# bcaitech1/p4-fr-sorry-math-but-love-you

Hardware: NVIDIA B200
Metric: EfficientSATRN greedy-decode images/sec (higher is better)
Workload: dtype bf16

## Files before the change

### p4-fr-sorry-math-but-love-you_b200/csrc/common.cuh

```cuda
#pragma once
#include <cuda_runtime.h>
#include <cuda_bf16.h>
#include <cuda_fp16.h>
#include <stdint.h>

#if defined(__CUDA_ARCH__) && (__CUDA_ARCH__ < 1000)
#error "frx is written for sm_100a (B200) only"
#endif

namespace frx {

enum Act : int { ACT_NONE = 0, ACT_RELU = 1, ACT_SILU = 2, ACT_SIGMOID = 3, ACT_GELU = 4 };

__device__ __forceinline__ float act_apply(float v, int act) {
  switch (act) {
    case ACT_RELU: return fmaxf(v, 0.f);
    case ACT_SILU: return v / (1.f + expf(-v));
    case ACT_SIGMOID: return 1.f / (1.f + expf(-v));
    case ACT_GELU: return 0.5f * v * (1.f + erff(v * 0.70710678118654752440f));
    default: return v;
  }
}

struct SmemOptIn {
  size_t bytes[64] = {};
  template <class Kernel>
  cudaError_t ensure(Kernel kernel, size_t smem, bool always = false) {
    int dev = 0;
    cudaGetDevice(&dev);
    dev &= 63;
    if ((!always && smem <= 48 * 1024) || (bytes[dev] != 0 && smem <= bytes[dev])) return cudaSuccess;
    cudaError_t e = cudaFuncSetAttribute(kernel, cudaFuncAttributeMaxDynamicSharedMemorySize, (int)smem);
    if (e == cudaSuccess) bytes[dev] = smem;
    return e;
  }
};

#ifndef FRX_ENC_FP16
#define FRX_ENC_FP16 1
#endif
#if FRX_ENC_FP16
typedef __half eh_t;
typedef __half2 eh2_t;
#define FRX_EH_PTX "f16"
__device__ __forceinline__ uint32_t eh2_pack(float lo, float hi) {
  uint32_t r;
  asm("cvt.rn.satfinite.f16x2.f32 %0, %1, %2;\n" : "=r"(r) : "f"(hi), "f"(lo));
  return r;
}
__device__ __forceinline__ eh_t eh_from_float(float f) {
  const uint32_t r = eh2_pack(f, 0.f);
  return __ushort_as_half((unsigned short)(r & 0xffffu));
}
__device__ __forceinline__ float eh_to_float(eh_t v) { return __half2float(v); }
__device__ __forceinline__ float2 eh2_unpack(uint32_t w) { return __half22float2(*reinterpret_cast<const __half2*>(&w)); }
#else
typedef __nv_bfloat16 eh_t;
typedef __nv_bfloat162 eh2_t;
#define FRX_EH_PTX "bf16"
__device__ __forceinline__ uint32_t eh2_pack(float lo, float hi) {
  __nv_bfloat162 t = __floats2bfloat162_rn(lo, hi);
  return *reinterpret_cast<uint32_t*>(&t);
}
__device__ __forceinline__ eh_t eh_from_float(float f) { return __float2bfloat16_rn(f); }
__device__ __forceinline__ float eh_to_float(eh_t v) { return __bfloat162float(v); }
__device__ __forceinline__ float2 eh2_unpack(uint32_t w) { return make_float2(__uint_as_float(w << 16), __uint_as_float(w & 0xffff0000u)); }
#endif

__device__ __forceinline__ float warp_sum(float v) {
#pragma unroll
  for (int o = 16; o > 0; o >>= 1) v += __shfl_xor_sync(0xffffffffu, v, o);
  return v;
}
__device__ __forceinline__ float warp_max(float v) {
#pragma unroll
  for (int o = 16; o > 0; o >>= 1) v = fmaxf(v, __shfl_xor_sync(0xffffffffu, v, o));
  return v;
}

struct GemmP {
  const float* A;
  const float* W;
  float* C;
  int M, N, K;
  int lda, ldc;
  int conv;
  int H, Wd, Cin, OH, OW, KH, KW, stride, pad_t, pad_l;
  const float* gate;
  int rows_per_img;
  const float* scale;
  const float* shift;
  int act;
  const float* res;
  int ldr;
  float* ws;
  long long ws_floats;
  int splitk, k_chunk;
};

struct DwP {
  const float* in;
  const float* w;
  const float* scale;
  const float* shift;
  float* out;
  int B, H, Wd, C, OH, OW, stride, pad_t, pad_l, act;
};

struct Seg {
  int n_begin, n_end;
  float* dst;
  long long row_stride;
  long long slot_stride;
};

struct DecGemmP {
  const float* A;
  const float* Wt;
  const float* bias;
  int M, N, K, lda;
  int act;
  const float* res;
  int ldr;
  const float* ln_g;
  const float* ln_b;
  float* a_norm_out;
  const int* row_slot;
  int nseg;
  Seg seg[4];
};

struct AttnP {
  const float* q;
  int ldq;
  const float* kcache;
  const float* vcache;
  int rows_per_img;
  int D;
  int n_hist;
  const int* hist_len;
  int causal_L;
  const unsigned char* key_mask;
  const int* chain;
  int chain_stride;
  const float* cur_k;
  const float* cur_v;
  int ld_cur;
  int q_per_img;
  float temperature;
  float* out;
  int ldo;
  int M;
  int heads;
};


struct BeamP {
  int B, V, bw, max_seq, T, cap, sos, eos, pad;
  double* hscore; int* hnode; int* hsize;
  int* nprev; int* ntok; int* nlen; double* nlogp; int* nkv; int* ncount;
  int *num_steps, *done, *endnode, *nexp, *cur_node;
  int *cur_tok, *pos, *slot, *active;
  int* chain;
  int* n_active;
  const float* logits;
  long long* out;
};

struct TcGemmP {
  const eh_t* A;
  const eh_t* W;
  void* C;
  int M, N, K, lda, ldw, ldc;
  int BN;
  int stages;
  int conv, H, Wd, Cin, OH, OW, KW, stride, pad_t, pad_l;
  const eh_t* Wpad;
  int im2col;
  const float* scale;
  const float* shift;
  int act;
  const void* res;
  int res_f32, ldr, out_f32;
};

struct SiftIds { int sos, eos, empty, lbrace, rbrace, underbar; };

constexpr int DEC_CLUSTER = 8;
constexpr int DEC_IMG = 8;
constexpr int DEC_FMAX = 1024;
constexpr int DEC_TMAX = 500;
constexpr int DEC_MAX_CLUSTERS = 32;

struct DecClusterLayer {
  const uint4 *w_o, *w_q2, *w_o2, *w_f0, *w_f1, *w_next;
  const float *b_o, *b_q2, *b_o2, *b_f0, *b_f1, *b_next;
  const float *ln1_g, *ln1_b, *ln2_g, *ln2_b, *ln3_g, *ln3_b;
};

struct DecClusterP {
  int B, steps, T, L, V, S, sos;
  int img_base;
  const uint4* w_first;
  const float* b_first;
  DecClusterLayer layer[4];
  const float* emb;
  const float* pe;
  __nv_bfloat16* kself;
  __nv_bfloat16* vself;
  const __nv_bfloat16* kcross;
  const __nv_bfloat16* vcross;
  float* logits;
  long long* tokens;
  const long long* forced;
  const int* hist_len;
  const int* chain;
  const int* slot;
  const int* first_tok32;
  const long long* first_tok64;
  const int* sift_flags;
  const int* sift_limit;
  SiftIds sift_ids;
  long long* prof;
};

}
```

### p4-fr-sorry-math-but-love-you_b200/csrc/kernels.h

```cpp
#pragma once
#include "common.cuh"

namespace frx {

void launch_stem_conv(const float* in, const float* w, const float* scale, const float* shift, float* out,
                      int B, int Cin, int H, int W, int OH, int OW, int Cout, cudaStream_t st);
void launch_direct_conv3x3(const float* in, const float* w, const float* scale, const float* shift, float* out, int B,
                           int Cin, int H, int W, int OH, int OW, int Cout, int stride, int pad, int act,
                           cudaStream_t st);
void launch_igemm_f32(const GemmP& p, cudaStream_t st);
void launch_dwconv_f32(const DwP& p, cudaStream_t st);
void launch_se_gate_f32(const float* x, const float* w1, const float* b1, const float* w2, const float* b2,
                        float* gate, int B, int HW, int C, int R, cudaStream_t st);
void launch_maxpool2_f32(const float* in, float* out, int B, int H, int W, int C, cudaStream_t st);
void launch_pe2d_f32(const float* x, const float* w0, const float* b0, const float* w1, const float* b1,
                     const float* peh, const float* pew, float* out, int B, int h, int w, int C,
                     cudaStream_t st);
void launch_layernorm_f32(const float* x, const float* res, const float* gamma, const float* beta, float* out,
                          int M, int C, int scramble_S, cudaStream_t st);
void launch_enc_attn_f32(const float* qkv, float* out, int B, int S, int D, int heads, cudaStream_t st);
void launch_dec_gemm_f32(const DecGemmP& p, cudaStream_t st);
void launch_dec_attn_f32(const AttnP& p, int head_dim, cudaStream_t st);
void launch_fill_i32(int* p, int v, int n, cudaStream_t st);
void launch_dec_embed_f32(const int* tok, const long long* tok64, int fixed_token, const float* emb,
                          const float* pe, int pos, const int* pos_arr, int pos_mod, float scale, float* x,
                          int M, int D, cudaStream_t st);
void launch_dec_argmax_embed(const float* logits, long long ld_logits, int V, long long* tokens_out,
                             long long ld_tok, const long long* forced, long long ld_forced, int* cur_tok,
                             const float* emb, const float* pe_next, float scale, float* x, int M, int D,
                             cudaStream_t st);


void launch_dec_sift_embed(float* logits, long long ld_logits, int V, long long* tokens_out, long long ld_tok, int4* state,
                           const int* flags, const int* limit, const SiftIds& ids, int* cur_tok, const float* emb,
                           const float* pe_next, float scale, float* x, int M, int D, cudaStream_t st);
void launch_sift_state_init(int4* state, int M, int sos, cudaStream_t st);
void launch_pad_mask(const long long* text, unsigned char* mask, int B, int L, int pad_id, cudaStream_t st);

void launch_swin_patch_embed(const float* img, const float* w, const float* bias, const float* g, const float* b,
                             const float* ape, float* out, int B, int IMGS, int R, int E, cudaStream_t st);
void launch_swin_window_attn(const float* qkv, const float* bias_table, float* out, int B, int R, int C, int heads, int ws,
                             int shift, cudaStream_t st);
bool launch_swin_window_attn_mma(const float* qkv, const float* bias_table, eh_t* out, int B, int R, int C, int heads,
                                 int ws, int shift, cudaStream_t st);
void launch_swin_patch_merge(const float* x, float* out, int B, int R, int C, cudaStream_t st);

void launch_beam_init(const BeamP& p, cudaStream_t st);
void launch_beam_select(const BeamP& p, cudaStream_t st);
void launch_beam_push(const BeamP& p, cudaStream_t st);
void launch_beam_finish(const BeamP& p, cudaStream_t st);

int launch_tc_igemm(TcGemmP p, cudaStream_t st);
int launch_tc_igemm_ws(TcGemmP p, int num_sms, cudaStream_t st);
void launch_pad_conv_weights(const eh_t* in, eh_t* out, long long rows, int Cin, cudaStream_t st);
void launch_h16_to_f32(const eh_t* in, float* out, long long n, cudaStream_t st);
void launch_f32_to_h16(const float* in, eh_t* out, long long n, cudaStream_t st);
void launch_stem_conv_bf16(const float* in, const float* w, const float* scale, const float* shift,
                           eh_t* out, int B, int Cin, int H, int W, int OH, int OW, int Cout, cudaStream_t st);
void launch_dwconv_bf16(const eh_t* in, const float* w, const float* scale, const float* shift,
                        eh_t* out, int B, int H, int W, int C, int OH, int OW, int stride, int pad_t,
                        int pad_l, int act, cudaStream_t st);
void launch_se_scale_bf16(eh_t* x, const float* w1, const float* b1, const float* w2, const float* b2,
                          int B, int HW, int C, int R, cudaStream_t st);
void launch_mbconv_dw_se_bf16(const eh_t* in, const float* w, const float* scale, const float* shift,
                              eh_t* out, float* mean, float* gate, const float* w1, const float* b1,
                              const float* w2, const float* b2, int B, int H, int W, int C, int OH, int OW, int stride,
                              int pad_t, int pad_l, int R, cudaStream_t st);
void launch_layernorm_bf16out(const float* x, const float* res, const float* gamma, const float* beta,
                              eh_t* out, int M, int C, int scramble_S, cudaStream_t st);
void launch_enc_attn_bf16out(const float* qkv, eh_t* out, int B, int S, int D, int heads, cudaStream_t st);
void launch_conv3x3_c24_bf16(const eh_t* in, const void* wfrag, const float* scale, const float* shift,
                             eh_t* out, int B, int H, int W, int add_res, cudaStream_t st);
void launch_lite_conv0_pool_bf16(const float* in, const float* w, const float* scale, const float* shift, eh_t* out,
                                 int B, int Cin, int H, int W, int Cout, cudaStream_t st);
void launch_maxpool2_bf16(const eh_t* in, eh_t* out, float* out_f32, int B, int H, int W, int C, cudaStream_t st);
bool launch_enc_attn_mma_bf16(const float* qkv, eh_t* out, int B, int S, int D, int heads, cudaStream_t st);

size_t dec_cluster_smem_bytes();
int launch_dec_cluster_bf16(const DecClusterP& p, cudaStream_t st);
int launch_dec_cluster_bf16_d128(const DecClusterP& p, cudaStream_t st);
int launch_dec_cluster_bf16_p2(const DecClusterP& p, cudaStream_t st);
int launch_dec_cluster_bf16_d512(const DecClusterP& p, cudaStream_t st);
void launch_cross_to_bf16(const float* src, __nv_bfloat16* kc, __nv_bfloat16* vc, int B, int S, int L, int Dm, int head_dim,
                          cudaStream_t st);

}
```

### p4-fr-sorry-math-but-love-you_b200/csrc/kernels_bf16.cu

```cuda
#include <cuda_fp16.h>

#include "common.cuh"
#include "kernels.h"

#ifndef FRX_DW_ACC32
#define FRX_DW_ACC32 2
#endif

namespace frx {

namespace {
__device__ __forceinline__ void unpack8(const uint4& u, float (&f)[8]) {
  const uint32_t w[4] = {u.x, u.y, u.z, u.w};
#pragma unroll
  for (int i = 0; i < 4; ++i) {
    const float2 t = eh2_unpack(w[i]);
    f[2 * i] = t.x;
    f[2 * i + 1] = t.y;
  }
}
__device__ __forceinline__ uint4 pack8(const float (&f)[8]) {
  uint32_t w[4];
#pragma unroll
  for (int i = 0; i < 4; ++i) w[i] = eh2_pack(f[2 * i], f[2 * i + 1]);
  return make_uint4(w[0], w[1], w[2], w[3]);
}
}

__global__ void __launch_bounds__(256) stem_conv_bf16_kernel(const float* __restrict__ in, const float* __restrict__ w,
                                                             const float* __restrict__ scale, const float* __restrict__ shift,
                                                             eh_t* __restrict__ out, int B, int Cin, int H, int W,
                                                             int OH, int OW, int Cout) {
  extern __shared__ float ws[];
  for (int i = threadIdx.x; i < Cout * Cin * 9; i += blockDim.x) ws[i] = w[i];
  float* ssc = ws + Cout * Cin * 9;
  float* ssh = ssc + Cout;
  for (int i = threadIdx.x; i < Cout; i += blockDim.x) { ssc[i] = scale[i]; ssh[i] = shift[i]; }
  __syncthreads();
  const int C8 = Cout / 8;
  long long total = (long long)B * OH * OW * C8;
  long long idx = (long long)blockIdx.x * blockDim.x + threadIdx.x;
  if (idx >= total) return;
  const int co0 = (int)(idx % C8) * 8;
  long long pix = idx / C8;
  const int ow = (int)(pix % OW), oh = (int)((pix / OW) % OH), n = (int)(pix / ((long long)OW * OH));
  float acc[8];
#pragma unroll
  for (int j = 0; j < 8; ++j) acc[j] = 0.f;
  for (int ci = 0; ci < Cin; ++ci) {
    const float* ip = in + (((long long)n * Cin + ci) * H + oh * 2) * W + ow * 2;
    float x[9];
#pragma unroll
    for (int kh = 0; kh < 3; ++kh)
#pragma unroll
      for (int kw = 0; kw < 3; ++kw) x[kh * 3 + kw] = __ldg(ip + kh * W + kw);
#pragma unroll
    for (int j = 0; j < 8; ++j) {
      const float* wp = ws + ((co0 + j) * Cin + ci) * 9;
#pragma unroll
      for (int t = 0; t < 9; ++t) acc[j] = fmaf(x[t], wp[t], acc[j]);
    }
  }
  float o[8];
#pragma unroll
  for (int j = 0; j < 8; ++j) o[j] = act_apply(acc[j] * ssc[co0 + j] + ssh[co0 + j], ACT_SILU);
  *reinterpret_cast<uint4*>(out + pix * Cout + co0) = pack8(o);
}

template <int COUT>
__global__ void __launch_bounds__(128) stem_conv_px_bf16_kernel(const float* __restrict__ in, const float* __restrict__ w,
                                                                const float* __restrict__ scale, const float* __restrict__ shift,
                                                                eh_t* __restrict__ out, int B, int Cin, int H, int W,
                                                                int OH, int OW) {
  extern __shared__ __align__(16) float ws[];
  const int taps = Cin * 9;
  for (int i = threadIdx.x; i < COUT * taps; i += blockDim.x) {
    const int co = i / taps, r = i - co * taps;
    ws[r * COUT + co] = w[i];
  }
  float* ssc = ws + COUT * taps;
  float* ssh = ssc + COUT;
  uint4* stage = reinterpret_cast<uint4*>(ws + ((COUT * taps + 2 * COUT + 3) & ~3));
  for (int i = threadIdx.x; i < COUT; i += blockDim.x) { ssc[i] = scale[i]; ssh[i] = shift[i]; }
  __syncthreads();
  const long long npix = (long long)B * OH * OW, pix0 = (long long)blockIdx.x * blockDim.x;
  const long long pix = min(pix0 + threadIdx.x, npix - 1);
  const int ow = (int)(pix % OW), oh = (int)((pix / OW) % OH), n = (int)(pix / ((long long)OW * OH));
  float acc[COUT];
#pragma unroll
  for (int j = 0; j < COUT; ++j) acc[j] = 0.f;
  for (int ci = 0; ci < Cin; ++ci) {
    const float* ip = in + (((long long)n * Cin + ci) * H + oh * 2) * W + ow * 2;
    float x[9];
#pragma unroll
    for (int kh = 0; kh < 3; ++kh)
#pragma unroll
      for (int kw = 0; kw < 3; ++kw) x[kh * 3 + kw] = __ldg(ip + kh * W + kw);
#pragma unroll
    for (int t = 0; t < 9; ++t) {
      const float4* wp = reinterpret_cast<const float4*>(ws + (ci * 9 + t) * COUT);
#pragma unroll
      for (int j = 0; j < COUT / 4; ++j) {
        const float4 wv = wp[j];
        acc[4 * j] = fmaf(x[t], wv.x, acc[4 * j]);
        acc[4 * j + 1] = fmaf(x[t], wv.y, acc[4 * j + 1]);
        acc[4 * j + 2] = fmaf(x[t], wv.z, acc[4 * j + 2]);
        acc[4 * j + 3] = fmaf(x[t], wv.w, acc[4 * j + 3]);
      }
    }
  }
#pragma unroll
  for (int g = 0; g < COUT / 8; ++g) {
    float o[8];
#pragma unroll
    for (int j = 0; j < 8; ++j) o[j] = act_apply(acc[g * 8 + j] * ssc[g * 8 + j] + ssh[g * 8 + j], ACT_SILU);
    stage[threadIdx.x * (COUT / 8) + g] = pack8(o);
  }
  __syncthreads();
  const long long cta_vecs = min((long long)blockDim.x, npix - pix0) * (COUT / 8);
  uint4* op = reinterpret_cast<uint4*>(out + pix0 * COUT);
  for (int i = threadIdx.x; i < cta_vecs; i += blockDim.x) op[i] = stage[i];
}

void launch_stem_conv_bf16(const float* in, const float* w, const float* scale, const float* shift,
                           eh_t* out, int B, int Cin, int H, int W, int OH, int OW, int Cout, cudaStream_t st) {
  if (Cout == 24) {
    const long long pixels = (long long)B * OH * OW;
    const int smem24 = ((24 * Cin * 9 + 2 * 24 + 3) & ~3) * sizeof(float) + 128 * 3 * 16;
    stem_conv_px_bf16_kernel<24><<<(unsigned)((pixels + 127) / 128), 128, smem24, st>>>(in, w, scale, shift, out, B, Cin, H, W, OH, OW);
    return;
  }
  long long total = (long long)B * OH * OW * (Cout / 8);
  int smem = (Cout * Cin * 9 + 2 * Cout) * sizeof(float);
  stem_conv_bf16_kernel<<<(unsigned)((total + 255) / 256), 256, smem, st>>>(in, w, scale, shift, out, B, Cin, H, W, OH, OW, Cout);
}

__global__ void __launch_bounds__(256) dwconv3x3_bf16_kernel(const eh_t* __restrict__ in, const float* __restrict__ w,
                                                             const float* __restrict__ scale, const float* __restrict__ shift,
                                                             eh_t* __restrict__ out, int B, int H, int W, int C, int OH,
                                                             int OW, int stride, int pad_t, int pad_l, int act) {
  const int C8 = C >> 3;
  long long total = (long long)B * OH * OW * C8;
  long long idx = (long long)blockIdx.x * blockDim.x + threadIdx.x;
  if (idx >= total) return;
  const int c = (int)(idx % C8) * 8;
  long long pix = idx / C8;
  const int ow = (int)(pix % OW), oh = (int)((pix / OW) % OH), n = (int)(pix / ((long long)OW * OH));
  float acc[8];
#pragma unroll
  for (int j = 0; j < 8; ++j) acc[j] = 0.f;
#pragma unroll
  for (int kh = 0; kh < 3; ++kh) {
    const int ih = oh * stride - pad_t + kh;
    if (ih < 0 || ih >= H) continue;
#pragma unroll
    for (int kw = 0; kw < 3; ++kw) {
      const int iw = ow * stride - pad_l + kw;
      if (iw < 0 || iw >= W) continue;
      float x[8];
      unpack8(__ldg(reinterpret_cast<const uint4*>(in + (((long long)n * H + ih) * W + iw) * C + c)), x);
      const float4 w0 = __ldg(reinterpret_cast<const float4*>(w + (kh * 3 + kw) * C + c));
      const float4 w1 = __ldg(reinterpret_cast<const float4*>(w + (kh * 3 + kw) * C + c + 4));
      acc[0] = fmaf(x[0], w0.x, acc[0]); acc[1] = fmaf(x[1], w0.y, acc[1]);
      acc[2] = fmaf(x[2], w0.z, acc[2]); acc[3] = fmaf(x[3], w0.w, acc[3]);
      acc[4] = fmaf(x[4], w1.x, acc[4]); acc[5] = fmaf(x[5], w1.y, acc[5]);
      acc[6] = fmaf(x[6], w1.z, acc[6]); acc[7] = fmaf(x[7], w1.w, acc[7]);
    }
  }
  float o[8];
#pragma unroll
  for (int j = 0; j < 8; ++j) o[j] = act_apply(acc[j] * __ldg(scale + c + j) + __ldg(shift + c + j), act);
  *reinterpret_cast<uint4*>(out + pix * C + c) = pack8(o);
}

void launch_dwconv_bf16(const eh_t* in, const float* w, const float* scale, const float* shift,
                        eh_t* out, int B, int H, int W, int C, int OH, int OW, int stride, int pad_t,
                        int pad_l, int act, cudaStream_t st) {
  long long total = (long long)B * OH * OW * (C / 8);
  dwconv3x3_bf16_kernel<<<(unsigned)((total + 255) / 256), 256, 0, st>>>(in, w, scale, shift, out, B, H, W, C, OH, OW,
                                                                        stride, pad_t, pad_l, act);
}

__global__ void __launch_bounds__(256) se_scale_bf16_kernel(eh_t* __restrict__ x, const float* __restrict__ w1,
                                                            const float* __restrict__ b1, const float* __restrict__ w2,
                                                            const float* __restrict__ b2, int HW, int C, int R) {
  extern __shared__ float sm[];
  float* mean = sm;
  float* red = sm + C;
  float* gate = red + R;
  const int n = blockIdx.x;
  eh_t* xp = x + (long long)n * HW * C;
  const float inv = 1.f / (float)HW;
  for (int c8 = threadIdx.x; c8 < C / 8; c8 += blockDim.x) {
    float s[8];
#pragma unroll
    for (int j = 0; j < 8; ++j) s[j] = 0.f;
    for (int q = 0; q < HW; ++q) {
      float v[8];
      unpack8(*reinterpret_cast<const uint4*>(xp + (long long)q * C + c8 * 8), v);
#pragma unroll
      for (int j = 0; j < 8; ++j) s[j] += v[j];
    }
#pragma unroll
    for (int j = 0; j < 8; ++j) mean[c8 * 8 + j] = s[j] * inv;
  }
  __syncthreads();
  const int warp = threadIdx.x >> 5, lane = threadIdx.x & 31;
  for (int r = warp; r < R; r += 8) {
    float s = 0.f;
    for (int c = lane; c < C; c += 32) s = fmaf(__ldg(w1 + (long long)r * C + c), mean[c], s);
    s = warp_sum(s);
    if (lane == 0) red[r] = act_apply(s + __ldg(b1 + r), ACT_SILU);
  }
  __syncthreads();
  for (int c = threadIdx.x; c < C; c += blockDim.x) {
    float s = __ldg(b2 + c);
    const float* wr = w2 + (long long)c * R;
    for (int r = 0; r < R; ++r) s = fmaf(__ldg(wr + r), red[r], s);
    gate[c] = 1.f / (1.f + expf(-s));
  }
  __syncthreads();
  for (int i = threadIdx.x; i < HW * (C / 8); i += blockDim.x) {
    const int c8 = i % (C / 8);
    uint4* ptr = reinterpret_cast<uint4*>(xp + (long long)(i / (C / 8)) * C + c8 * 8);
    float v[8];
    unpack8(*ptr, v);
#pragma unroll
    for (int j = 0; j < 8; ++j) v[j] *= gate[c8 * 8 + j];
    *ptr = pack8(v);
  }
}

void launch_se_scale_bf16(eh_t* x, const float* w1, const float* b1, const float* w2, const float* b2,
                          int B, int HW, int C, int R, cudaStream_t st) {
  se_scale_bf16_kernel<<<B, 256, (2 * C + R) * sizeof(float), st>>>(x, w1, b1, w2, b2, HW, C, R);
}


__global__ void __launch_bounds__(256) dwconv_se_mean_kernel(const eh_t* __restrict__ in, const float* __restrict__ w,
                                                             const float* __restrict__ scale, const float* __restrict__ shift,
                                                             eh_t* __restrict__ out, float* __restrict__ mean,
                                                             int H, int W, int C, int OH, int OW, int stride, int pad_t,
                                                             int pad_l, const float* __restrict__ se_w1,
                                                             const float* __restrict__ se_w2, int se_floats) {
  extern __shared__ __align__(16) unsigned char dw_smem[];
  {
    const long long line = ((long long)(blockIdx.y * gridDim.x + blockIdx.x) * blockDim.x + threadIdx.x) * 32;
    if (line < se_floats) {
      asm volatile("prefetch.global.L2 [%0];\n" ::"l"(se_w1 + line));
      asm volatile("prefetch.global.L2 [%0];\n" ::"l"(se_w2 + line));
    }
  }
  uint4* tile = reinterpret_cast<uint4*>(dw_smem);
  float (*red)[64 + 1] = reinterpret_cast<float (*)[64 + 1]>(dw_smem + (size_t)H * W * 8 * 16);
  float* wsm = reinterpret_cast<float*>(dw_smem + (size_t)H * W * 8 * 16 + 32 * 65 * sizeof(float));
  const int n = blockIdx.x, c0 = blockIdx.y * 64;
  const int cg = threadIdx.x & 7, pl = threadIdx.x >> 3;
  const int c = c0 + cg * 8;
  const bool c_ok = c < C;
  const eh_t* ip = in + (long long)n * H * W * C;
  for (int i = threadIdx.x; i < H * W * 8; i += 256) {
    const int px = i >> 3, g = i & 7;
    tile[i] = (c0 + g * 8 < C) ? __ldg(reinterpret_cast<const uint4*>(ip + (long long)px * C + c0 + g * 8)) : make_uint4(0u, 0u, 0u, 0u);
  }
  float sum[8];
#pragma unroll
  for (int j = 0; j < 8; ++j) sum[j] = 0.f;
  for (int i = threadIdx.x; i < 11 * 64; i += 256) {
    const int t = i >> 6, cc = c0 + (i & 63);
    const float* src = t < 9 ? w + t * C : (t == 9 ? scale : shift);
    wsm[i] = cc < C ? __ldg(src + cc) : 0.f;
  }
  __syncthreads();
  auto ld8s = [&](int t, float (&dst)[8]) {
    const float4 a = *reinterpret_cast<const float4*>(wsm + t * 64 + cg * 8);
    const float4 b4 = *reinterpret_cast<const float4*>(wsm + t * 64 + cg * 8 + 4);
    dst[0] = a.x; dst[1] = a.y; dst[2] = a.z; dst[3] = a.w; dst[4] = b4.x; dst[5] = b4.y; dst[6] = b4.z; dst[7] = b4.w;
  };
  float sc[8], sh[8];
  ld8s(9, sc);
  ld8s(10, sh);
  eh_t* op = out + (long long)n * OH * OW * C;
  if (c_ok) {
    for (int px = pl; px < OH * OW; px += 32) {
      const int oh = px / OW, ow = px - oh * OW;
      float acc[8];
#pragma unroll
      for (int j = 0; j < 8; ++j) acc[j] = 0.f;
#pragma unroll
      for (int kh = 0; kh < 3; ++kh) {
        const int ih = oh * stride - pad_t + kh;
#pragma unroll
        for (int kw = 0; kw < 3; ++kw) {
          const int iw = ow * stride - pad_l + kw;
          if (ih >= 0 && ih < H && iw >= 0 && iw < W) {
            float x[8], wv[8];
            unpack8(tile[(ih * W + iw) * 8 + cg], x);
            ld8s(kh * 3 + kw, wv);
#pragma unroll
            for (int j = 0; j < 8; ++j) acc[j] = fmaf(x[j], wv[j], acc[j]);
          }
        }
      }
      float o[8];
#pragma unroll
      for (int j = 0; j < 8; ++j) {
        const float v = fmaf(acc[j], sc[j], sh[j]);
        o[j] = __fdividef(v, 1.f + __expf(-v));
      }
      const uint4 packed = pack8(o);
      *reinterpret_cast<uint4*>(op + (long long)px * C + c) = packed;
      float back[8];
      unpack8(packed, back);
#pragma unroll
      for (int j = 0; j < 8; ++j) sum[j] += back[j];
    }
  }
#pragma unroll
  for (int j = 0; j < 8; ++j) red[pl][cg * 8 + j] = sum[j];
  __syncthreads();
  if (threadIdx.x < 64 && c0 + threadIdx.x < C) {
    float s = 0.f;
#pragma unroll
    for (int i = 0; i < 32; ++i) s += red[i][threadIdx.x];
    mean[(long long)n * C + c0 + threadIdx.x] = s / (float)(OH * OW);
  }
}

template <int CH>
__global__ void __launch_bounds__(CH * 4) dwconv4_se_mean_kernel(const eh_t* __restrict__ in, const float* __restrict__ w,
                                                                 const float* __restrict__ scale, const float* __restrict__ shift,
                                                                 eh_t* __restrict__ out, float* __restrict__ mean,
                                                                 int H, int W, int C, int OH, int OW, int stride, int pad_t,
                                                                 int pad_l, const float* __restrict__ se_w1,
                                                                 const float* __restrict__ se_w2, int se_floats) {
  constexpr int NT = CH * 4, G8 = CH / 8, G4 = CH / 4;
  extern __shared__ __align__(16) unsigned char dw_smem[];
  {
    const long long line = ((long long)(blockIdx.y * gridDim.x + blockIdx.x) * NT + threadIdx.x) * 32;
    if (line < se_floats) {
      asm volatile("prefetch.global.L2 [%0];\n" ::"l"(se_w1 + line));
      asm volatile("prefetch.global.L2 [%0];\n" ::"l"(se_w2 + line));
    }
  }
  uint4* tile = reinterpret_cast<uint4*>(dw_smem);
  float (*red)[CH + 1] = reinterpret_cast<float (*)[CH + 1]>(dw_smem + (size_t)H * W * G8 * 16);
  const int n = blockIdx.x, c0 = blockIdx.y * CH;
  const eh_t* ip = in + (long long)n * H * W * C;
  for (int i = threadIdx.x; i < H * W * G8; i += NT) {
    const int px = i / G8, g = i - px * G8;
    uint4 v = make_uint4(0u, 0u, 0u, 0u);
    if (c0 + g * 8 < C) {
#if FRX_ENC_FP16
      v = __ldg(reinterpret_cast<const uint4*>(ip + (long long)px * C + c0 + g * 8));
#else
      float x[8];
      unpack8(__ldg(reinterpret_cast<const uint4*>(ip + (long long)px * C + c0 + g * 8)), x);
      const __half2 h0 = __floats2half2_rn(x[0], x[1]), h1 = __floats2half2_rn(x[2], x[3]);
      const __half2 h2 = __floats2half2_rn(x[4], x[5]), h3 = __floats2half2_rn(x[6], x[7]);
      v = make_uint4(*reinterpret_cast<const uint32_t*>(&h0), *reinterpret_cast<const uint32_t*>(&h1),
                     *reinterpret_cast<const uint32_t*>(&h2), *reinterpret_cast<const uint32_t*>(&h3));
#endif
    }
    tile[i] = v;
  }
  const int cg = threadIdx.x % G4, pl = threadIdx.x / G4;
  const int c = c0 + cg * 4;
  const bool c_ok = c < C;
#if FRX_DW_ACC32
  float4 wt[9], sc, sh;
#if FRX_DW_ACC32 == 2
  __half2 wh[9][2];
#endif
  {
    const float4 z = make_float4(0.f, 0.f, 0.f, 0.f);
#pragma unroll
    for (int t = 0; t < 9; ++t) wt[t] = c_ok ? __ldg(reinterpret_cast<const float4*>(w + t * C + c)) : z;
#if FRX_DW_ACC32 == 2
#pragma unroll
    for (int t = 0; t < 9; ++t) { wh[t][0] = __floats2half2_rn(wt[t].x, wt[t].y); wh[t][1] = __floats2half2_rn(wt[t].z, wt[t].w); }
#endif
    sc = c_ok ? __ldg(reinterpret_cast<const float4*>(scale + c)) : z;
    sh = c_ok ? __ldg(reinterpret_cast<const float4*>(shift + c)) : z;
  }
  __syncthreads();
  const uint2* tile2 = reinterpret_cast<const uint2*>(tile);
  float sum[4] = {0.f, 0.f, 0.f, 0.f};
  eh_t* op = out + (long long)n * OH * OW * C;
  if (c_ok) {
    for (int px = pl; px < OH * OW; px += 16) {
      const int oh = px / OW, ow = px - oh * OW;
      float4 acc = make_float4(0.f, 0.f, 0.f, 0.f);
#pragma unroll
      for (int kh = 0; kh < 3; ++kh) {
        const int ih = oh * stride - pad_t + kh;
#if FRX_DW_ACC32 == 2
        __half2 r0 = __floats2half2_rn(0.f, 0.f), r1 = r0;
#pragma unroll
        for (int kw = 0; kw < 3; ++kw) {
          const int iw = ow * stride - pad_l + kw;
          if (ih >= 0 && ih < H && iw >= 0 && iw < W) {
            const uint2 u = tile2[(ih * W + iw) * G4 + cg];
            r0 = __hfma2(*reinterpret_cast<const __half2*>(&u.x), wh[kh * 3 + kw][0], r0);
            r1 = __hfma2(*reinterpret_cast<const __half2*>(&u.y), wh[kh * 3 + kw][1], r1);
          }
        }
        const float2 a = __half22float2(r0), b = __half22float2(r1);
        acc.x += a.x; acc.y += a.y; acc.z += b.x; acc.w += b.y;
#else
#pragma unroll
        for (int kw = 0; kw < 3; ++kw) {
          const int iw = ow * stride - pad_l + kw;
          if (ih >= 0 && ih < H && iw >= 0 && iw < W) {
            const uint2 u = tile2[(ih * W + iw) * G4 + cg];
            const float2 a = __half22float2(*reinterpret_cast<const __half2*>(&u.x)), b = __half22float2(*reinterpret_cast<const __half2*>(&u.y));
            const float4 ww = wt[kh * 3 + kw];
            acc.x = fmaf(a.x, ww.x, acc.x); acc.y = fmaf(a.y, ww.y, acc.y); acc.z = fmaf(b.x, ww.z, acc.z); acc.w = fmaf(b.y, ww.w, acc.w);
          }
        }
#endif
      }
      float2 f0 = make_float2(fmaf(acc.x, sc.x, sh.x), fmaf(acc.y, sc.y, sh.y)), f1 = make_float2(fmaf(acc.z, sc.z, sh.z), fmaf(acc.w, sc.w, sh.w));
      f0.x = __fdividef(f0.x, 1.f + __expf(-f0.x)); f0.y = __fdividef(f0.y, 1.f + __expf(-f0.y));
      f1.x = __fdividef(f1.x, 1.f + __expf(-f1.x)); f1.y = __fdividef(f1.y, 1.f + __expf(-f1.y));
#else
  __half2 wt[9][2], sc[2], sh[2];
  {
    const float4 z = make_float4(0.f, 0.f, 0.f, 0.f);
#pragma unroll
    for (int t = 0; t < 9; ++t) {
      const float4 f = c_ok ? __ldg(reinterpret_cast<const float4*>(w + t * C + c)) : z;
      wt[t][0] = __floats2half2_rn(f.x, f.y); wt[t][1] = __floats2half2_rn(f.z, f.w);
    }
    const float4 a = c_ok ? __ldg(reinterpret_cast<const float4*>(scale + c)) : z;
    const float4 d = c_ok ? __ldg(reinterpret_cast<const float4*>(shift + c)) : z;
    sc[0] = __floats2half2_rn(a.x, a.y); sc[1] = __floats2half2_rn(a.z, a.w);
    sh[0] = __floats2half2_rn(d.x, d.y); sh[1] = __floats2half2_rn(d.z, d.w);
  }
  const __half2 half_ = __floats2half2_rn(0.5f, 0.5f);
  __syncthreads();
  const uint2* tile2 = reinterpret_cast<const uint2*>(tile);
  float sum[4] = {0.f, 0.f, 0.f, 0.f};
  eh_t* op = out + (long long)n * OH * OW * C;
  if (c_ok) {
    for (int px = pl; px < OH * OW; px += 16) {
      const int oh = px / OW, ow = px - oh * OW;
      __half2 acc0 = __floats2half2_rn(0.f, 0.f), acc1 = acc0;
#pragma unroll
      for (int kh = 0; kh < 3; ++kh) {
        const int ih = oh * stride - pad_t + kh;
#pragma unroll
        for (int kw = 0; kw < 3; ++kw) {
          const int iw = ow * stride - pad_l + kw;
          if (ih >= 0 && ih < H && iw >= 0 && iw < W) {
            const uint2 u = tile2[(ih * W + iw) * G4 + cg];
            acc0 = __hfma2(*reinterpret_cast<const __half2*>(&u.x), wt[kh * 3 + kw][0], acc0);
            acc1 = __hfma2(*reinterpret_cast<const __half2*>(&u.y), wt[kh * 3 + kw][1], acc1);
          }
        }
      }
      const __half2 v0 = __hfma2(acc0, sc[0], sh[0]), v1 = __hfma2(acc1, sc[1], sh[1]);
      const __half2 o0 = __hmul2(v0, __hfma2(h2tanh_approx(__hmul2(v0, half_)), half_, half_));
      const __half2 o1 = __hmul2(v1, __hfma2(h2tanh_approx(__hmul2(v1, half_)), half_, half_));
      const float2 f0 = __half22float2(o0), f1 = __half22float2(o1);
#endif
      uint2 packed;
      packed.x = eh2_pack(f0.x, f0.y);
      packed.y = eh2_pack(f1.x, f1.y);
      *reinterpret_cast<uint2*>(op + (long long)px * C + c) = packed;
      const float2 b0 = eh2_unpack(packed.x), b1 = eh2_unpack(packed.y);
      sum[0] += b0.x; sum[1] += b0.y; sum[2] += b1.x; sum[3] += b1.y;
    }
  }
#pragma unroll
  for (int j = 0; j < 4; ++j) red[pl][cg * 4 + j] = sum[j];
  __syncthreads();
  if (threadIdx.x < CH && c0 + threadIdx.x < C) {
    float s2 = 0.f;
#pragma unroll
    for (int i = 0; i < 16; ++i) s2 += red[i][threadIdx.x];
    mean[(long long)n * C + c0 + threadIdx.x] = s2 / (float)(OH * OW);
  }
}

constexpr int SE_IMGS = 4;
constexpr int SE_ROWS = 4;
__global__ void __launch_bounds__(512, 1) se_fc_kernel(const float* __restrict__ mean, const float* __restrict__ w1,
                                                       const float* __restrict__ b1, const float* __restrict__ w2,
                                                       const float* __restrict__ b2, float* __restrict__ gate, int B, int C,
                                                       int R) {
  extern __shared__ float sm[];
  float* mv = sm;
  float* red = sm + SE_IMGS * C;
  const int n0 = blockIdx.x * SE_IMGS;
  for (int i = threadIdx.x; i < SE_IMGS * C; i += blockDim.x) {
    const int im = i / C;
    mv[i] = n0 + im < B ? mean[(long long)n0 * C + i] : 0.f;
  }
  __syncthreads();
  const int warp = threadIdx.x >> 5, lane = threadIdx.x & 31;
  const int nwarps = blockDim.x >> 5;
  for (int r0 = warp * SE_ROWS; r0 < R; r0 += nwarps * SE_ROWS) {
    float s[SE_ROWS][SE_IMGS];
#pragma unroll
    for (int j = 0; j < SE_ROWS; ++j)
#pragma unroll
      for (int im = 0; im < SE_IMGS; ++im) s[j][im] = 0.f;
#pragma unroll 3
    for (int c4 = lane; c4 < C / 4; c4 += 32) {
      float4 wv[SE_ROWS], m4[SE_IMGS];
#pragma unroll
      for (int j = 0; j < SE_ROWS; ++j)
        wv[j] = r0 + j < R ? __ldg(reinterpret_cast<const float4*>(w1 + (long long)(r0 + j) * C) + c4) : make_float4(0.f, 0.f, 0.f, 0.f);
#pragma unroll
      for (int im = 0; im < SE_IMGS; ++im) m4[im] = *reinterpret_cast<const float4*>(mv + im * C + c4 * 4);
#pragma unroll
      for (int j = 0; j < SE_ROWS; ++j)
#pragma unroll
        for (int im = 0; im < SE_IMGS; ++im)
          s[j][im] = fmaf(wv[j].x, m4[im].x, fmaf(wv[j].y, m4[im].y, fmaf(wv[j].z, m4[im].z, fmaf(wv[j].w, m4[im].w, s[j][im]))));
    }
#pragma unroll
    for (int j = 0; j < SE_ROWS; ++j)
#pragma unroll
      for (int im = 0; im < SE_IMGS; ++im) {
        const float t = warp_sum(s[j][im]);
        if (lane == 0 && r0 + j < R) red[im * R + r0 + j] = act_apply(t + __ldg(b1 + r0 + j), ACT_SILU);
      }
  }
  __syncthreads();
  for (int c = blockIdx.y * blockDim.x + threadIdx.x; c < C; c += gridDim.y * blockDim.x) {
    float s[SE_IMGS];
    const float bb = __ldg(b2 + c);
#pragma unroll
    for (int im = 0; im < SE_IMGS; ++im) s[im] = bb;
#pragma unroll 32
    for (int r = 0; r < R; ++r) {
      const float wv = __ldg(w2 + (long long)r * C + c);
#pragma unroll
      for (int im = 0; im < SE_IMGS; ++im) s[im] = fmaf(wv, red[im * R + r], s[im]);
    }
#pragma unroll
    for (int im = 0; im < SE_IMGS; ++im)
      if (n0 + im < B) gate[(long long)(n0 + im) * C + c] = 1.f / (1.f + expf(-s[im]));
  }
}

__global__ void __launch_bounds__(256) se_apply_kernel(eh_t* __restrict__ x, const float* __restrict__ gate,
                                                       long long total8, int HW, int C) {
  long long i = (long long)blockIdx.x * blockDim.x + threadIdx.x;
  if (i >= total8) return;
  const int C8 = C >> 3;
  const int c = (int)(i % C8) * 8;
  const long long n = i / ((long long)C8 * HW);
  uint4* ptr = reinterpret_cast<uint4*>(x) + i;
  float v[8];
  unpack8(*ptr, v);
  const float4 g0 = __ldg(reinterpret_cast<const float4*>(gate + n * C + c));
  const float4 g1 = __ldg(reinterpret_cast<const float4*>(gate + n * C + c + 4));
  v[0] *= g0.x; v[1] *= g0.y; v[2] *= g0.z; v[3] *= g0.w;
  v[4] *= g1.x; v[5] *= g1.y; v[6] *= g1.z; v[7] *= g1.w;
  *ptr = pack8(v);
}

void launch_mbconv_dw_se_bf16(const eh_t* in, const float* w, const float* scale, const float* shift,
                              eh_t* out, float* mean, float* gate, const float* w1, const float* b1,
                              const float* w2, const float* b2, int B, int H, int W, int C, int OH, int OW, int stride,
                              int pad_t, int pad_l, int R, cudaStream_t st) {
  dim3 g(B, (C + 63) / 64);
  const size_t smem = (size_t)H * W * 8 * 16 + 32 * 65 * sizeof(float) + 11 * 64 * sizeof(float);
  static SmemOptIn opt;
  opt.ensure(dwconv_se_mean_kernel, smem);
  if (C % 8 == 0) {
    constexpr int CH = 32;
    const size_t sm4 = (size_t)H * W * (CH / 8) * 16 + 16 * (CH + 1) * sizeof(float);
    static SmemOptIn opt4;
    opt4.ensure(dwconv4_se_mean_kernel<CH>, sm4);
    dwconv4_se_mean_kernel<CH><<<dim3(B, (C + CH - 1) / CH), CH * 4, sm4, st>>>(in, w, scale, shift, out, mean, H, W, C, OH, OW,
                                                                             stride, pad_t, pad_l, w1, w2, R * C);
  } else {
    dwconv_se_mean_kernel<<<g, 256, smem, st>>>(in, w, scale, shift, out, mean, H, W, C, OH, OW, stride, pad_t, pad_l, w1, w2, R * C);
  }
  se_fc_kernel<<<dim3((B + SE_IMGS - 1) / SE_IMGS, 2), 512, SE_IMGS * (C + R) * sizeof(float), st>>>(mean, w1, b1, w2, b2, gate, B, C, R);
  long long total8 = (long long)B * OH * OW * (C / 8);
  se_apply_kernel<<<(unsigned)((total8 + 255) / 256), 256, 0, st>>>(out, gate, total8, OH * OW, C);
}

__device__ __forceinline__ uint32_t pack2(float lo, float hi) {
  return eh2_pack(lo, hi);
}
__device__ __forceinline__ void mma16816(float (&c)[4], const uint32_t (&a)[4], uint32_t b0, uint32_t b1) {
  asm("mma.sync.aligned.m16n8k16.row.col.f32." FRX_EH_PTX "." FRX_EH_PTX ".f32 {%0,%1,%2,%3}, {%4,%5,%6,%7}, {%8,%9}, {%0,%1,%2,%3};\n"
      : "+f"(c[0]), "+f"(c[1]), "+f"(c[2]), "+f"(c[3])
      : "r"(a[0]), "r"(a[1]), "r"(a[2]), "r"(a[3]), "r"(b0), "r"(b1));
}

template <int S>
__global__ void __launch_bounds__(S * 2) enc_attn_mma_kernel(const float* __restrict__ qkv,
                                                             eh_t* __restrict__ out,
                                                             int D, int heads, float inv_temp) {
  constexpr int HD = 64, NT = S / 8;
  const int b = blockIdx.x / heads, hh = blockIdx.x % heads;
  const int warp = threadIdx.x >> 5, lane = threadIdx.x & 31, gid = lane >> 2, tig = lane & 3;
  const int ld = 3 * D;
  const float* qb = qkv + (long long)b * S * ld + hh * HD;
  const int i0 = warp * 16;
  float sacc[NT][4];
#pragma unroll
  for (int nt = 0; nt < NT; ++nt)
#pragma unroll
    for (int e = 0; e < 4; ++e) sacc[nt][e] = 0.f;
#pragma unroll
  for (int ks = 0; ks < 4; ++ks) {
    const float* q0 = qb + (long long)(i0 + gid) * ld + 16 * ks + 2 * tig;
    const float* q1 = q0 + 8 * ld;
    const float2 a00 = __ldg(reinterpret_cast<const float2*>(q0)), a10 = __ldg(reinterpret_cast<const float2*>(q1));
    const float2 a01 = __ldg(reinterpret_cast<const float2*>(q0 + 8)), a11 = __ldg(reinterpret_cast<const float2*>(q1 + 8));
    const uint32_t a[4] = {pack2(a00.x, a00.y), pack2(a10.x, a10.y), pack2(a01.x, a01.y), pack2(a11.x, a11.y)};
#pragma unroll
    for (int nt = 0; nt < NT; ++nt) {
      const float* kp = qb + D + (long long)(8 * nt + gid) * ld + 16 * ks + 2 * tig;
      const float2 k0 = __ldg(reinterpret_cast<const float2*>(kp)), k1 = __ldg(reinterpret_cast<const float2*>(kp + 8));
      mma16816(sacc[nt], a, pack2(k0.x, k0.y), pack2(k1.x, k1.y));
    }
  }
  float mx0 = -INFINITY, mx1 = -INFINITY;
#pragma unroll
  for (int nt = 0; nt < NT; ++nt) {
#pragma unroll
    for (int e = 0; e < 4; ++e) sacc[nt][e] *= inv_temp;
    mx0 = fmaxf(mx0, fmaxf(sacc[nt][0], sacc[nt][1]));
    mx1 = fmaxf(mx1, fmaxf(sacc[nt][2], sacc[nt][3]));
  }
  mx0 = fmaxf(mx0, __shfl_xor_sync(0xffffffffu, mx0, 1)); mx0 = fmaxf(mx0, __shfl_xor_sync(0xffffffffu, mx0, 2));
  mx1 = fmaxf(mx1, __shfl_xor_sync(0xffffffffu, mx1, 1)); mx1 = fmaxf(mx1, __shfl_xor_sync(0xffffffffu, mx1, 2));
  float sum0 = 0.f, sum1 = 0.f;
#pragma unroll
  for (int nt = 0; nt < NT; ++nt) {
    sacc[nt][0] = __expf(sacc[nt][0] - mx0); sacc[nt][1] = __expf(sacc[nt][1] - mx0);
    sacc[nt][2] = __expf(sacc[nt][2] - mx1); sacc[nt][3] = __expf(sacc[nt][3] - mx1);
    sum0 += sacc[nt][0] + sacc[nt][1];
    sum1 += sacc[nt][2] + sacc[nt][3];
  }
  sum0 += __shfl_xor_sync(0xffffffffu, sum0, 1); sum0 += __shfl_xor_sync(0xffffffffu, sum0, 2);
  sum1 += __shfl_xor_sync(0xffffffffu, sum1, 1); sum1 += __shfl_xor_sync(0xffffffffu, sum1, 2);
  float oacc[8][4];
#pragma unroll
  for (int n = 0; n < 8; ++n)
#pragma unroll
    for (int e = 0; e < 4; ++e) oacc[n][e] = 0.f;
#pragma unroll
  for (int kk = 0; kk < S / 16; ++kk) {
    const uint32_t a[4] = {pack2(sacc[2 * kk][0], sacc[2 * kk][1]), pack2(sacc[2 * kk][2], sacc[2 * kk][3]),
                           pack2(sacc[2 * kk + 1][0], sacc[2 * kk + 1][1]), pack2(sacc[2 * kk + 1][2], sacc[2 * kk + 1][3])};
    const float* vp = qb + 2 * D + (long long)(16 * kk + 2 * tig) * ld + gid;
#pragma unroll
    for (int n = 0; n < 8; ++n) {
      const float v00 = __ldg(vp + 8 * n), v01 = __ldg(vp + ld + 8 * n);
      const float v10 = __ldg(vp + 8 * ld + 8 * n), v11 = __ldg(vp + 9 * ld + 8 * n);
      mma16816(oacc[n], a, pack2(v00, v01), pack2(v10, v11));
    }
  }
  const float r0 = __fdividef(1.f, sum0), r1 = __fdividef(1.f, sum1);
  eh_t* o0 = out + ((long long)b * S + i0 + gid) * D + hh * HD + 2 * tig;
  eh_t* o1 = o0 + (long long)8 * D;
#pragma unroll
  for (int n = 0; n < 8; ++n) {
    *reinterpret_cast<uint32_t*>(o0 + 8 * n) = pack2(oacc[n][0] * r0, oacc[n][1] * r0);
    *reinterpret_cast<uint32_t*>(o1 + 8 * n) = pack2(oacc[n][2] * r1, oacc[n][3] * r1);
  }
}

bool launch_enc_attn_mma_bf16(const float* qkv, eh_t* out, int B, int S, int D, int heads, cudaStream_t st) {
  if (D / heads != 64 || D % heads != 0) return false;
  const float inv_temp = 1.f / sqrtf((float)D);
  if (S == 32) enc_attn_mma_kernel<32><<<B * heads, 64, 0, st>>>(qkv, out, D, heads, inv_temp);
  else if (S == 128) enc_attn_mma_kernel<128><<<B * heads, 256, 0, st>>>(qkv, out, D, heads, inv_temp);
  else return false;
  return true;
}

constexpr int C24 = 24, C24_TH = 8, C24_TW = 32, C24_KS = 14;

__global__ void __launch_bounds__(256) conv3x3_c24_mma_kernel(const eh_t* __restrict__ in, const uint2* __restrict__ wfrag,
                                                              const float* __restrict__ scale, const float* __restrict__ shift,
                                                              eh_t* __restrict__ out, int H, int W, int add_res) {
  constexpr int PW = C24_TW + 2, PH = C24_TH + 2;
  __shared__ __align__(16) eh_t halo[PH * PW * C24];
  __shared__ uint2 wsm[C24_KS * 3 * 32];
  const int tiles_x = (W + C24_TW - 1) / C24_TW, tiles_y = (H + C24_TH - 1) / C24_TH;
  const int n = blockIdx.x / (tiles_x * tiles_y), t = blockIdx.x % (tiles_x * tiles_y);
  const int y0 = (t / tiles_x) * C24_TH, x0 = (t % tiles_x) * C24_TW;
  const eh_t* ip = in + (long long)n * H * W * C24;
  for (int i = threadIdx.x; i < PH * PW * 3; i += 256) {
    const int pix = i / 3, ch = i - pix * 3;
    const int py = pix / PW, px = pix - py * PW;
    const int y = y0 + py - 1, x = x0 + px - 1;
    uint4 v = make_uint4(0u, 0u, 0u, 0u);
    if (y >= 0 && y < H && x >= 0 && x < W) v = __ldg(reinterpret_cast<const uint4*>(ip + ((long long)y * W + x) * C24) + ch);
    reinterpret_cast<uint4*>(halo)[i] = v;
  }
  for (int i = threadIdx.x; i < C24_KS * 3 * 32; i += 256) wsm[i] = __ldg(wfrag + i);
  __syncthreads();
  const int warp = threadIdx.x >> 5, lane = threadIdx.x & 31, gid = lane >> 2, tig = lane & 3;
  float acc[2][3][4];
#pragma unroll
  for (int mt = 0; mt < 2; ++mt)
#pragma unroll
    for (int nt = 0; nt < 3; ++nt)
#pragma unroll
      for (int e = 0; e < 4; ++e) acc[mt][nt][e] = 0.f;
  const uint32_t* hw = reinterpret_cast<const uint32_t*>(halo);
#pragma unroll
  for (int s = 0; s < C24_KS; ++s) {
    const int klo = 16 * s, khi = 16 * s + 8;
    const int tap_lo = klo / C24, ch_lo = klo % C24, tap_hi = khi / C24, ch_hi = khi % C24;
    uint32_t a[2][4];
#pragma unroll
    for (int mt = 0; mt < 2; ++mt) {
      const int px = mt * 16 + gid;
      const int p_lo = ((warp + tap_lo / 3) * PW + px + tap_lo % 3) * 12 + (ch_lo >> 1) + tig;
      a[mt][0] = hw[p_lo];
      a[mt][1] = hw[p_lo + 8 * 12];
      if (tap_hi < 9) {
        const int p_hi = ((warp + tap_hi / 3) * PW + px + tap_hi % 3) * 12 + (ch_hi >> 1) + tig;
        a[mt][2] = hw[p_hi];
        a[mt][3] = hw[p_hi + 8 * 12];
      } else {
        a[mt][2] = 0u; a[mt][3] = 0u;
      }
    }
#pragma unroll
    for (int nt = 0; nt < 3; ++nt) {
      const uint2 b = wsm[(s * 3 + nt) * 32 + lane];
      mma16816(acc[0][nt], a[0], b.x, b.y);
      mma16816(acc[1][nt], a[1], b.x, b.y);
    }
  }
  const int y = y0 + warp;
  if (y >= H) return;
  eh_t* op = out + ((long long)n * H + y) * W * C24;
#pragma unroll
  for (int nt = 0; nt < 3; ++nt) {
    const int ch = nt * 8 + 2 * tig;
    const float s0 = __ldg(scale + ch), s1 = __ldg(scale + ch + 1), h0 = __ldg(shift + ch), h1 = __ldg(shift + ch + 1);
#pragma unroll
    for (int mt = 0; mt < 2; ++mt)
#pragma unroll
      for (int hr = 0; hr < 2; ++hr) {
        const int px = mt * 16 + gid + hr * 8, x = x0 + px;
        if (x >= W) continue;
        float v0 = fmaf(acc[mt][nt][2 * hr], s0, h0), v1 = fmaf(acc[mt][nt][2 * hr + 1], s1, h1);
        v0 = __fdividef(v0, 1.f + __expf(-v0));
        v1 = __fdividef(v1, 1.f + __expf(-v1));
        if (add_res) {
          const uint32_t r = hw[((warp + 1) * PW + px + 1) * 12 + (ch >> 1)];
          const float2 rf = eh2_unpack(r);
          v0 += rf.x;
          v1 += rf.y;
        }
        *reinterpret_cast<uint32_t*>(op + (long long)x * C24 + ch) = pack2(v0, v1);
      }
  }
}

void launch_conv3x3_c24_bf16(const eh_t* in, const void* wfrag, const float* scale, const float* shift,
                             eh_t* out, int B, int H, int W, int add_res, cudaStream_t st) {
  const int tiles = ((W + C24_TW - 1) / C24_TW) * ((H + C24_TH - 1) / C24_TH);
  conv3x3_c24_mma_kernel<<<B * tiles, 256, 0, st>>>(in, reinterpret_cast<const uint2*>(wfrag), scale, shift, out, H, W, add_res);
}

__global__ void __launch_bounds__(256) lite_conv0_pool_bf16_kernel(const float* __restrict__ in, const float* __restrict__ w,
                                                                   const float* __restrict__ scale, const float* __restrict__ shift,
                                                                   eh_t* __restrict__ out, int B, int Cin, int H, int W, int Cout) {
  extern __shared__ float ws0[];
  for (int i = threadIdx.x; i < Cout * Cin * 9; i += blockDim.x) ws0[i] = w[i];
  float* ssc = ws0 + Cout * Cin * 9;
  float* ssh = ssc + Cout;
  for (int i = threadIdx.x; i < Cout; i += blockDim.x) { ssc[i] = scale[i]; ssh[i] = shift[i]; }
  __syncthreads();
  const int OH = H / 2, OW = W / 2, C8 = Cout / 8;
  const long long total = (long long)B * OH * OW * C8;
  const long long idx = (long long)blockIdx.x * blockDim.x + threadIdx.x;
  if (idx >= total) return;
  const int co0 = (int)(idx % C8) * 8;
  const long long pix = idx / C8;
  const int ow = (int)(pix % OW), oh = (int)((pix / OW) % OH), n = (int)(pix / ((long long)OW * OH));
  float acc[4][8];
#pragma unroll
  for (int q = 0; q < 4; ++q)
#pragma unroll
    for (int j = 0; j < 8; ++j) acc[q][j] = 0.f;
  for (int ci = 0; ci < Cin; ++ci) {
    float x[4][4];
#pragma unroll
    for (int a = 0; a < 4; ++a)
#pragma unroll
      for (int b = 0; b < 4; ++b) {
        const int ih = 2 * oh - 1 + a, iw = 2 * ow - 1 + b;
        x[a][b] = (ih >= 0 && ih < H && iw >= 0 && iw < W) ? __ldg(in + (((long long)n * Cin + ci) * H + ih) * W + iw) : 0.f;
      }
#pragma unroll
    for (int j = 0; j < 8; ++j) {
      const float* wp = ws0 + ((co0 + j) * Cin + ci) * 9;
#pragma unroll
      for (int kh = 0; kh < 3; ++kh)
#pragma unroll
        for (int kw = 0; kw < 3; ++kw) {
          const float wv = wp[kh * 3 + kw];
          acc[0][j] = fmaf(x[kh][kw], wv, acc[0][j]);
          acc[1][j] = fmaf(x[kh][kw + 1], wv, acc[1][j]);
          acc[2][j] = fmaf(x[kh + 1][kw], wv, acc[2][j]);
          acc[3][j] = fmaf(x[kh + 1][kw + 1], wv, acc[3][j]);
        }
    }
  }
  float o[8];
#pragma unroll
  for (int j = 0; j < 8; ++j) {
    const float s = ssc[co0 + j], t = ssh[co0 + j];
    const float m = fmaxf(fmaxf(fmaf(acc[0][j], s, t), fmaf(acc[1][j], s, t)), fmaxf(fmaf(acc[2][j], s, t), fmaf(acc[3][j], s, t)));
    o[j] = fmaxf(m, 0.f);
  }
  *reinterpret_cast<uint4*>(out + pix * Cout + co0) = pack8(o);
}

template <int KS, int Cout>
__global__ void __launch_bounds__(256) lite_conv0_pool_mma_kernel(const float* __restrict__ in, const float* __restrict__ w,
                                                                  const float* __restrict__ scale, const float* __restrict__ shift,
                                                                  eh_t* __restrict__ out, int B, int Cin, int H, int W) {
  constexpr int NT = Cout / 8;
  const int lane = threadIdx.x & 31, gid = lane >> 2, tig = lane & 3;
  const int OH = H / 2, OW = W / 2, K = 9 * Cin;
  const long long tiles = (long long)B * OH * (OW / 4);
  const long long tile = (long long)blockIdx.x * 8 + (threadIdx.x >> 5);
  if (tile >= tiles) return;
  uint32_t bf[KS][NT][2];
#pragma unroll
  for (int ks = 0; ks < KS; ++ks)
#pragma unroll
    for (int nt = 0; nt < NT; ++nt)
#pragma unroll
      for (int h2 = 0; h2 < 2; ++h2) {
        const int k = 16 * ks + 8 * h2 + 2 * tig, n = 8 * nt + gid;
        const float lo = k < K ? __ldg(w + (long long)n * K + k) : 0.f, hi = k + 1 < K ? __ldg(w + (long long)n * K + k + 1) : 0.f;
        bf[ks][nt][h2] = pack2(lo, hi);
      }
  const int owq = (int)(tile % (OW / 4));
  const long long t2 = tile / (OW / 4);
  const int oh = (int)(t2 % OH), n = (int)(t2 / OH);
  const int pp = gid & 3, pos0 = gid >> 2;
  const int ow = owq * 4 + pp;
  const float* img = in + (long long)n * Cin * H * W;
  auto patch = [&](int pos, int k) -> float {
    if (k >= K) return 0.f;
    const int ci = k / 9, tap = k - ci * 9, kh = tap / 3, kw = tap - kh * 3;
    const int ih = 2 * oh + (pos >> 1) + kh - 1, iw = 2 * ow + (pos & 1) + kw - 1;
    return (ih >= 0 && ih < H && iw >= 0 && iw < W) ? __ldg(img + ((long long)ci * H + ih) * W + iw) : 0.f;
  };
  float acc[NT][4];
#pragma unroll
  for (int nt = 0; nt < NT; ++nt)
#pragma unroll
    for (int e = 0; e < 4; ++e) acc[nt][e] = 0.f;
#pragma unroll
  for (int ks = 0; ks < KS; ++ks) {
    const int k0 = 16 * ks + 2 * tig;
    const uint32_t a[4] = {pack2(patch(pos0, k0), patch(pos0, k0 + 1)), pack2(patch(pos0 + 2, k0), patch(pos0 + 2, k0 + 1)),
                           pack2(patch(pos0, k0 + 8), patch(pos0, k0 + 9)), pack2(patch(pos0 + 2, k0 + 8), patch(pos0 + 2, k0 + 9))};
#pragma unroll
    for (int nt = 0; nt < NT; ++nt) mma16816(acc[nt], a, bf[ks][nt][0], bf[ks][nt][1]);
  }
  eh_t* op = out + (((long long)n * OH + oh) * OW + ow) * Cout;
#pragma unroll
  for (int nt = 0; nt < NT; ++nt) {
    const int ch = 8 * nt + 2 * tig;
    const float s0 = __ldg(scale + ch), s1 = __ldg(scale + ch + 1), t0 = __ldg(shift + ch), t1 = __ldg(shift + ch + 1);
    float m0 = fmaxf(fmaf(acc[nt][0], s0, t0), fmaf(acc[nt][2], s0, t0));
    float m1 = fmaxf(fmaf(acc[nt][1], s1, t1), fmaf(acc[nt][3], s1, t1));
    m0 = fmaxf(m0, __shfl_xor_sync(0xffffffffu, m0, 16));
    m1 = fmaxf(m1, __shfl_xor_sync(0xffffffffu, m1, 16));
    if (gid < 4) *reinterpret_cast<uint32_t*>(op + ch) = pack2(fmaxf(m0, 0.f), fmaxf(m1, 0.f));
  }
}

void launch_lite_conv0_pool_bf16(const float* in, const float* w, const float* scale, const float* shift, eh_t* out,
                                 int B, int Cin, int H, int W, int Cout, cudaStream_t st) {
  if ((Cout == 64 || Cout == 128) && Cin <= 3 && (W / 2) % 4 == 0 && H % 2 == 0) {
    const long long tiles = (long long)B * (H / 2) * (W / 2 / 4);
    const unsigned grid = (unsigned)((tiles + 7) / 8);
    if (Cout == 64) {
      if (Cin == 1) lite_conv0_pool_mma_kernel<1, 64><<<grid, 256, 0, st>>>(in, w, scale, shift, out, B, Cin, H, W);
      else lite_conv0_pool_mma_kernel<2, 64><<<grid, 256, 0, st>>>(in, w, scale, shift, out, B, Cin, H, W);
    } else {
      if (Cin == 1) lite_conv0_pool_mma_kernel<1, 128><<<grid, 256, 0, st>>>(in, w, scale, shift, out, B, Cin, H, W);
      else lite_conv0_pool_mma_kernel<2, 128><<<grid, 256, 0, st>>>(in, w, scale, shift, out, B, Cin, H, W);
    }
    return;
  }
  const long long total = (long long)B * (H / 2) * (W / 2) * (Cout / 8);
  const int smem = (Cout * Cin * 9 + 2 * Cout) * sizeof(float);
  lite_conv0_pool_bf16_kernel<<<(unsigned)((total + 255) / 256), 256, smem, st>>>(in, w, scale, shift, out, B, Cin, H, W, Cout);
}

__global__ void __launch_bounds__(256) maxpool2_bf16_kernel(const eh_t* __restrict__ in, eh_t* __restrict__ out,
                                                            float* __restrict__ out_f32, int B, int H, int W, int C) {
  const int OH = H / 2, OW = W / 2, C8 = C / 8;
  const long long total = (long long)B * OH * OW * C8;
  const long long idx = (long long)blockIdx.x * blockDim.x + threadIdx.x;
  if (idx >= total) return;
  const int c = (int)(idx % C8) * 8;
  const long long pix = idx / C8;
  const int ow = (int)(pix % OW), oh = (int)((pix / OW) % OH), n = (int)(pix / ((long long)OW * OH));
  const eh_t* base = in + (((long long)n * H + oh * 2) * W + ow * 2) * C + c;
  float a[8], b[8], d[8], e[8], o[8];
  unpack8(__ldg(reinterpret_cast<const uint4*>(base)), a);
  unpack8(__ldg(reinterpret_cast<const uint4*>(base + C)), b);
  unpack8(__ldg(reinterpret_cast<const uint4*>(base + (long long)W * C)), d);
  unpack8(__ldg(reinterpret_cast<const uint4*>(base + (long long)W * C + C)), e);
#pragma unroll
  for (int j = 0; j < 8; ++j) o[j] = fmaxf(fmaxf(a[j], b[j]), fmaxf(d[j], e[j]));
  if (out_f32) {
    float4* op = reinterpret_cast<float4*>(out_f32 + pix * C + c);
    op[0] = make_float4(o[0], o[1], o[2], o[3]);
    op[1] = make_float4(o[4], o[5], o[6], o[7]);
  } else {
    *reinterpret_cast<uint4*>(out + pix * C + c) = pack8(o);
  }
}

void launch_maxpool2_bf16(const eh_t* in, eh_t* out, float* out_f32, int B, int H, int W, int C, cudaStream_t st) {
  const long long total = (long long)B * (H / 2) * (W / 2) * (C / 8);
  maxpool2_bf16_kernel<<<(unsigned)((total + 255) / 256), 256, 0, st>>>(in, out, out_f32, B, H, W, C);
}

}
```

### p4-fr-sorry-math-but-love-you_b200/csrc/kernels_tc.cu

```cuda
#include <cuda.h>
#include <cuda_fp16.h>
#include <cudaTypedefs.h>

#include <cstdio>
#include <cstdlib>

#include "common.cuh"
#include "kernels.h"

namespace frx {

namespace {

constexpr int TC_BM = 128;
constexpr int TC_BK = 64;
constexpr int TC_STAGES = 3;
constexpr int TC_A_BYTES = TC_BM * TC_BK * 2;

__device__ __forceinline__ uint32_t smem_u32(const void* p) { return (uint32_t)__cvta_generic_to_shared(p); }

__device__ __forceinline__ void cp_async16(uint32_t dst, const void* src, uint32_t src_bytes) {
  asm volatile("cp.async.cg.shared.global [%0], [%1], 16, %2;\n" ::"r"(dst), "l"(src), "r"(src_bytes) : "memory");
}
__device__ __forceinline__ void cp_async_commit() { asm volatile("cp.async.commit_group;\n" ::: "memory"); }
// ... 233 lines not shown
  __shared__ uint32_t tmem_base_s;

  const int tid = threadIdx.x, warp = tid >> 5, lane = tid & 31;
  const int BN = p.BN;
  const uint32_t b_bytes = (uint32_t)BN * (TC_BK * 2);
  const uint32_t stage_bytes = TC_A_BYTES + b_bytes;
  const int NS = p.stages;
  const uint32_t smem0 = (smem_u32(dyn_smem) + 1023u) & ~1023u;
  const int m0 = blockIdx.x * TC_BM, n0 = blockIdx.y * BN;
  const int KB = (p.K + TC_BK - 1) / TC_BK;

  if (warp == 0) {
    asm volatile("tcgen05.alloc.cta_group::1.sync.aligned.shared::cta.b32 [%0], %1;\n" ::"r"(smem_u32(&tmem_base_s)), "n"(NCOLS) : "memory");
    asm volatile("tcgen05.relinquish_alloc_permit.cta_group::1.sync.aligned;\n" ::: "memory");
  }
  if (tid == 32) {
#pragma unroll
    for (int s = 0; s < TC_STAGES; ++s) mbar_init(&mma_done[s], 1);
    mbar_init(&acc_done, 1);
    asm volatile("fence.mbarrier_init.release.cluster;\n" ::: "memory");
  }
  tc_fence_before();
  __syncthreads();
  tc_fence_after();
  const uint32_t tmem = tmem_base_s;

  const int c = tid & 7, rbase = tid >> 3;
  const eh_t* a_ptr[4];
  int a_ih0[4], a_iw0[4];
  bool a_ok[4];
#pragma unroll
  for (int i = 0; i < 4; ++i) {
    const int m = m0 + rbase + 32 * i;
    a_ok[i] = m < p.M;
    a_ih0[i] = a_iw0[i] = 0;
    a_ptr[i] = p.A;
    if (a_ok[i]) {
      if (p.conv) {
        const int ow = m % p.OW;
        const int t = m / p.OW;
        const int oh = t % p.OH;
        const int n = t / p.OH;
        a_ptr[i] = p.A + (size_t)n * p.H * p.Wd * p.Cin;
        a_ih0[i] = oh * p.stride - p.pad_t;
        a_iw0[i] = ow * p.stride - p.pad_l;
      } else {
        a_ptr[i] = p.A + (size_t)m * p.lda;
      }
    }
  }
  const int nb_rows = (BN + 31) / 32;

  auto load_stage = [&](int kb, int stage) {
    const uint32_t sa = smem0 + (uint32_t)stage * stage_bytes;
    const uint32_t sb = sa + TC_A_BYTES;
    const int k = kb * TC_BK + c * 8;
    int tap = 0, ci = k, kh = 0, kw = 0;
    if (p.conv) {
      tap = k / p.Cin;
      ci = k - tap * p.Cin;
      kh = tap / p.KW;
      kw = tap - kh * p.KW;
    }
#pragma unroll
    for (int i = 0; i < 4; ++i) {
      const int row = rbase + 32 * i;
      const uint32_t dst = sa + (uint32_t)(row >> 3) * 1024u + (uint32_t)(row & 7) * 128u + (uint32_t)((c ^ (row & 7)) << 4);
      const eh_t* src = p.A;
      uint32_t bytes = 0;
      if (a_ok[i] && k < p.K) {
        if (p.conv) {
          const int ih = a_ih0[i] + kh, iw = a_iw0[i] + kw;
          if (ih >= 0 && ih < p.H && iw >= 0 && iw < p.Wd) {
            src = a_ptr[i] + ((size_t)ih * p.Wd + iw) * p.Cin + ci;
            bytes = 16;
          }
        } else {
          src = a_ptr[i] + k;
          bytes = 16;
        }
      }
      cp_async16(dst, src, bytes);
    }
    for (int j = 0; j < nb_rows; ++j) {
      const int row = rbase + 32 * j;
      if (row < BN) {
        const uint32_t dst = sb + (uint32_t)(row >> 3) * 1024u + (uint32_t)(row & 7) * 128u + (uint32_t)((c ^ (row & 7)) << 4);
        const int n = n0 + row;
        const bool ok = n < p.N && k < p.K;
        cp_async16(dst, ok ? p.W + (size_t)n * p.ldw + k : p.W, ok ? 16u : 0u);
      }
    }
  };

  for (int s = 0; s < NS - 1; ++s) {
    if (s < KB) load_stage(s, s);
    cp_async_commit();
  }
  const uint32_t idesc = make_idesc(BN);
  for (int kb = 0; kb < KB; ++kb) {
    if (NS == 3) cp_async_wait<1>(); else cp_async_wait<0>();
    asm volatile("fence.proxy.async.shared::cta;\n" ::: "memory");
    __syncthreads();
    const int stage = kb % NS;
    if (tid == 0) {
      tc_fence_after();
      const uint32_t sa = smem0 + (uint32_t)stage * stage_bytes;
      const uint64_t adesc = make_smem_desc(sa), bdesc = make_smem_desc(sa + TC_A_BYTES);
#pragma unroll
      for (int j = 0; j < TC_BK / 16; ++j)
        umma_f16(tmem, adesc + (uint64_t)(2 * j), bdesc + (uint64_t)(2 * j), idesc, (kb | j) ? 1u : 0u);
      umma_commit(&mma_done[stage]);
      if (kb == KB - 1) umma_commit(&acc_done);
    }
    const int nk = kb + NS - 1;
    if (nk < KB) {
      if (kb >= 1) mbar_wait(&mma_done[(kb - 1) % NS], (uint32_t)(((kb - 1) / NS) & 1));
      load_stage(nk, nk % NS);
    }
    cp_async_commit();
  }
  cp_async_wait<0>();
  mbar_wait(&acc_done, 0);
  tc_fence_after();

  {
    const int q = warp & 3;
    const int m = m0 + q * 32 + lane;
    const bool m_ok = m < p.M;
    for (int cc = (warp >> 2); cc * 16 < BN; cc += 2) {
      uint32_t r[16];
      tmem_ld16(tmem + ((uint32_t)(q * 32) << 16) + (uint32_t)(cc * 16), r);
      const int nb = n0 + cc * 16;
      if (m_ok && nb < p.N) epilogue_store16<false>(p, r, m, nb);
    }
  }
  tc_fence_before();
  __syncthreads();
  if (warp == 0) {
    asm volatile("tcgen05.dealloc.cta_group::1.sync.aligned.b32 %0, %1;\n" ::"r"(tmem), "n"(NCOLS) : "memory");
  }
}


constexpr int WS_STAGES = 4;
constexpr int WS_LAG = 2;
constexpr int WS_PROD_WARPS = 8;
constexpr int WS_EPI_WARPS = 8;
constexpr int WS_MMA_WARP = WS_PROD_WARPS + WS_EPI_WARPS;
constexpr int WS_TMA_WARP = WS_MMA_WARP + 1;
constexpr int WS_THREADS = (WS_TMA_WARP + 1) * 32;
constexpr int WS_PROD_THREADS = WS_PROD_WARPS * 32;
constexpr int WS_ROWS_PER_PASS = WS_PROD_THREADS / 8;
constexpr int WS_A_PASSES = TC_BM / WS_ROWS_PER_PASS;

template <int NCOLS, bool GELU>
__global__ void __launch_bounds__(WS_THREADS, NCOLS >= 256 ? 1 : 2) tc_igemm_ws_kernel(const TcGemmP p, const __grid_constant__ CUtensorMap tmA,
                                                                  const __grid_constant__ CUtensorMap tmW) {
  extern __shared__ unsigned char dyn_smem[];
  __shared__ __align__(8) uint64_t full_bar[WS_STAGES], empty_bar[WS_STAGES], acc_full[2], acc_empty[2];
  __shared__ uint32_t tmem_base_s;

  const int tid = threadIdx.x, warp = tid >> 5, lane = tid & 31;
  const int BN = p.BN;
  const uint32_t stage_bytes = TC_A_BYTES + (uint32_t)BN * (TC_BK * 2);
  const uint32_t smem0 = (smem_u32(dyn_smem) + 1023u) & ~1023u;
  const int KB = p.im2col ? p.KW * p.KW : (p.K + TC_BK - 1) / TC_BK;
  const int tiles_n = (p.N + BN - 1) / BN;
  const int tiles_m = (p.M + TC_BM - 1) / TC_BM;
  const int num_tiles = tiles_m * tiles_n;
  const bool gather = p.conv && !p.im2col;

  if (warp == WS_MMA_WARP) {
    asm volatile("tcgen05.alloc.cta_group::1.sync.aligned.shared::cta.b32 [%0], %1;\n" ::"r"(smem_u32(&tmem_base_s)), "n"(NCOLS) : "memory");
    asm volatile("tcgen05.relinquish_alloc_permit.cta_group::1.sync.aligned;\n" ::: "memory");
  }
  if (tid == 0) {
#pragma unroll
    for (int s = 0; s < WS_STAGES; ++s) { mbar_init(&full_bar[s], (gather ? WS_PROD_THREADS : 0) + 1); mbar_init(&empty_bar[s], 1); }
    mbar_init(&acc_full[0], 1); mbar_init(&acc_full[1], 1);
    const int epi_threads = (WS_EPI_WARPS + (gather ? 0 : WS_PROD_WARPS)) * 32;
    mbar_init(&acc_empty[0], epi_threads); mbar_init(&acc_empty[1], epi_threads);
    asm volatile("fence.mbarrier_init.release.cluster;\n" ::: "memory");
  }
  tc_fence_before();
  __syncthreads();
  tc_fence_after();
  const uint32_t tmem = tmem_base_s;

  if (gather ? warp < WS_PROD_WARPS : warp == WS_TMA_WARP) {
    const bool tma_thread = gather ? tid == 0 : lane == 0;
    const uint32_t tma_bytes = (uint32_t)BN * (TC_BK * 2) + (gather ? 0u : (uint32_t)TC_A_BYTES);
    if (!gather && !tma_thread) {
    } else {
    const int c = tid & 7, rbase = tid >> 3;
    int it = 0;
    for (int tile = blockIdx.x; tile < num_tiles; tile += gridDim.x) {
      const int m0 = (tile / tiles_n) * TC_BM, n0 = (tile % tiles_n) * BN;
      const eh_t* a_ptr[WS_A_PASSES];
      int a_ih0[WS_A_PASSES], a_iw0[WS_A_PASSES];
      bool a_ok[WS_A_PASSES];
      int bw = 0, bh = 0, bn = 0;
      if (p.im2col) {
        const int ow = m0 % p.OW, tq = m0 / p.OW;
        bw = ow * p.stride - p.pad_l;
        bh = (tq % p.OH) * p.stride - p.pad_t;
        bn = tq / p.OH;
      }
      if (gather) {
#pragma unroll
        for (int i = 0; i < WS_A_PASSES; ++i) {
          const int m = m0 + rbase + WS_ROWS_PER_PASS * i;
          a_ok[i] = m < p.M;
          a_ih0[i] = a_iw0[i] = 0;
          a_ptr[i] = p.A;
          if (a_ok[i]) {
            const int ow = m % p.OW;
            const int tq = m / p.OW;
            const int oh = tq % p.OH;
            const int n = tq / p.OH;
            a_ptr[i] = p.A + (size_t)n * p.H * p.Wd * p.Cin;
            a_ih0[i] = oh * p.stride - p.pad_t;
            a_iw0[i] = ow * p.stride - p.pad_l;
          }
        }
      }
      for (int kb = 0; kb < KB; ++kb, ++it) {
        const int stage = it % WS_STAGES;
        mbar_wait(&empty_bar[stage], (uint32_t)(((it / WS_STAGES) & 1) ^ 1));
        const uint32_t sa = smem0 + (uint32_t)stage * stage_bytes, sb = sa + TC_A_BYTES;
        if (tma_thread) {
          mbar_arrive_expect_tx(&full_bar[stage], tma_bytes);
          tma_load_2d(sb, &tmW, kb * TC_BK, n0, &full_bar[stage]);
          if (p.im2col) tma_load_im2col(sa, &tmA, 0, bw, bh, bn, (uint16_t)(kb % p.KW), (uint16_t)(kb / p.KW), &full_bar[stage]);
          else if (!p.conv) tma_load_2d(sa, &tmA, kb * TC_BK, m0, &full_bar[stage]);
        }
        if (gather) {
          const int k = kb * TC_BK + c * 8;
          const int tap = k / p.Cin;
          const int ci = k - tap * p.Cin;
          const int kh = tap / p.KW;
          const int kw = tap - kh * p.KW;
#pragma unroll
          for (int i = 0; i < WS_A_PASSES; ++i) {
            const int row = rbase + WS_ROWS_PER_PASS * i;
            const uint32_t dst = sa + (uint32_t)(row >> 3) * 1024u + (uint32_t)(row & 7) * 128u + (uint32_t)((c ^ (row & 7)) << 4);
            const eh_t* src = p.A;
            uint32_t bytes = 0;
            if (a_ok[i] && k < p.K) {
              const int ih = a_ih0[i] + kh, iw = a_iw0[i] + kw;
              if (ih >= 0 && ih < p.H && iw >= 0 && iw < p.Wd) {
                src = a_ptr[i] + ((size_t)ih * p.Wd + iw) * p.Cin + ci;
                bytes = 16;
              }
            }
            cp_async16(dst, src, bytes);
          }
          cp_async_commit();
          if (it >= WS_LAG) {
            cp_async_wait<WS_LAG>();
            asm volatile("fence.proxy.async.shared::cta;\n" ::: "memory");
            mbar_arrive(&full_bar[(it - WS_LAG) % WS_STAGES]);
          }
        }
      }
    }
    if (gather) {
      cp_async_wait<0>();
      asm volatile("fence.proxy.async.shared::cta;\n" ::: "memory");
      for (int j = (it >= WS_LAG ? it - WS_LAG : 0); j < it; ++j) mbar_arrive(&full_bar[j % WS_STAGES]);
    }
    }
  } else if (warp == WS_MMA_WARP) {
    if (lane == 0) {
      const uint32_t idesc = make_idesc(BN);
      int it = 0, ti = 0;
      for (int tile = blockIdx.x; tile < num_tiles; tile += gridDim.x, ++ti) {
        const int a = ti & 1;
        mbar_wait(&acc_empty[a], (uint32_t)(((ti >> 1) & 1) ^ 1));
        tc_fence_after();
        const uint32_t tacc = tmem + (uint32_t)(a * (NCOLS / 2));
        for (int kb = 0; kb < KB; ++kb, ++it) {
          const int stage = it % WS_STAGES;
          mbar_wait(&full_bar[stage], (uint32_t)((it / WS_STAGES) & 1));
          tc_fence_after();
          const uint32_t sa = smem0 + (uint32_t)stage * stage_bytes;
          const uint64_t adesc = make_smem_desc(sa), bdesc = make_smem_desc(sa + TC_A_BYTES);
#pragma unroll
          for (int j = 0; j < TC_BK / 16; ++j)
            umma_f16(tacc, adesc + (uint64_t)(2 * j), bdesc + (uint64_t)(2 * j), idesc, (kb | j) ? 1u : 0u);
          umma_commit(&empty_bar[stage]);
          if (kb == KB - 1) umma_commit(&acc_full[a]);
        }
      }
    }
  } else if (warp < WS_MMA_WARP) {
    const int q = warp & 3;
    const int nsub = (WS_EPI_WARPS + (gather ? 0 : WS_PROD_WARPS)) / 4;
    const int sub = (gather ? warp - WS_PROD_WARPS : warp) >> 2;
    int ti = 0;
    for (int tile = blockIdx.x; tile < num_tiles; tile += gridDim.x, ++ti) {
      const int a = ti & 1;
      const int m0 = (tile / tiles_n) * TC_BM, n0 = (tile % tiles_n) * BN;
      mbar_wait(&acc_full[a], (uint32_t)((ti >> 1) & 1));
      tc_fence_after();
      const int m = m0 + q * 32 + lane;
      const bool m_ok = m < p.M;
      const uint32_t tacc = tmem + (uint32_t)(a * (NCOLS / 2)) + ((uint32_t)(q * 32) << 16);
      for (int cc = sub; cc * 16 < BN; cc += nsub) {
        uint32_t r[16];
        tmem_ld16(tacc + (uint32_t)(cc * 16), r);
        const int nb = n0 + cc * 16;
        if (m_ok && nb < p.N) epilogue_store16<GELU>(p, r, m, nb);
      }
      tc_fence_before();
      mbar_arrive(&acc_empty[a]);
    }
  }
  tc_fence_before();
  __syncthreads();
  if (warp == WS_MMA_WARP) {
    asm volatile("tcgen05.dealloc.cta_group::1.sync.aligned.b32 %0, %1;\n" ::"r"(tmem), "n"(NCOLS) : "memory");
  }
}

static int tc_pick_bn(int N) {
  if (N <= 256) return (N + 15) / 16 * 16;
  for (int bn = 256; bn >= 128; bn -= 16)
    if (N % bn == 0) return bn;
  return 256;
}

template <int NCOLS>
static int tc_launch(const TcGemmP& p, cudaStream_t st) {
  const size_t smem = (size_t)p.stages * (TC_A_BYTES + (size_t)p.BN * TC_BK * 2) + 1024;
  static SmemOptIn opt;
  {
    cudaError_t e = opt.ensure(tc_igemm_kernel<NCOLS>, smem, true);
    if (e != cudaSuccess) return (int)e;
  }
  dim3 grid((p.M + TC_BM - 1) / TC_BM, (p.N + p.BN - 1) / p.BN);
  tc_igemm_kernel<NCOLS><<<grid, 256, smem, st>>>(p);
  return 0;
}

static PFN_cuTensorMapEncodeTiled_v12000 tensor_map_encoder() {
  static PFN_cuTensorMapEncodeTiled_v12000 fn = nullptr;
  if (!fn) {
    void* ptr = nullptr;
    cudaDriverEntryPointQueryResult qres;
    if (cudaGetDriverEntryPoint("cuTensorMapEncodeTiled", &ptr, cudaEnableDefault, &qres) == cudaSuccess &&
        qres == cudaDriverEntryPointSuccess)
      fn = reinterpret_cast<PFN_cuTensorMapEncodeTiled_v12000>(ptr);
  }
  return fn;
}

static int make_tmap_2d(CUtensorMap* tm, const void* base, long long rows, long long cols, long long ld, int box_rows) {
  PFN_cuTensorMapEncodeTiled_v12000 enc = tensor_map_encoder();
  if (!enc) return (int)cudaErrorNotSupported;
  cuuint64_t dims[2] = {(cuuint64_t)cols, (cuuint64_t)rows};
  cuuint64_t strides[1] = {(cuuint64_t)ld * 2};
  cuuint32_t box[2] = {(cuuint32_t)TC_BK, (cuuint32_t)box_rows};
  cuuint32_t estr[2] = {1, 1};
  CUresult r = enc(tm, (FRX_ENC_FP16 ? CU_TENSOR_MAP_DATA_TYPE_FLOAT16 : CU_TENSOR_MAP_DATA_TYPE_BFLOAT16), 2, const_cast<void*>(base), dims, strides, box, estr,
                   CU_TENSOR_MAP_INTERLEAVE_NONE, CU_TENSOR_MAP_SWIZZLE_128B, CU_TENSOR_MAP_L2_PROMOTION_L2_128B,
                   CU_TENSOR_MAP_FLOAT_OOB_FILL_NONE);
  return r == CUDA_SUCCESS ? 0 : (int)cudaErrorInvalidValue;
}

static PFN_cuTensorMapEncodeIm2col_v12000 im2col_map_encoder() {
  static PFN_cuTensorMapEncodeIm2col_v12000 fn = nullptr;
  if (!fn) {
    void* ptr = nullptr;
    cudaDriverEntryPointQueryResult qres;
    if (cudaGetDriverEntryPoint("cuTensorMapEncodeIm2col", &ptr, cudaEnableDefault, &qres) == cudaSuccess &&
        qres == cudaDriverEntryPointSuccess)
      fn = reinterpret_cast<PFN_cuTensorMapEncodeIm2col_v12000>(ptr);
  }
  return fn;
}

static int make_tmap_im2col(CUtensorMap* tm, const TcGemmP& p) {
  PFN_cuTensorMapEncodeIm2col_v12000 enc = im2col_map_encoder();
  if (!enc) return (int)cudaErrorNotSupported;
  const int B = p.M / (p.OH * p.OW), k = p.KW;
  const int pad_r = (p.OW - 1) * p.stride + k - p.Wd - p.pad_l, pad_b = (p.OH - 1) * p.stride + k - p.H - p.pad_t;
  cuuint64_t dims[4] = {(cuuint64_t)p.Cin, (cuuint64_t)p.Wd, (cuuint64_t)p.H, (cuuint64_t)B};
  cuuint64_t strides[3] = {(cuuint64_t)p.Cin * 2, (cuuint64_t)p.Wd * p.Cin * 2, (cuuint64_t)p.H * p.Wd * p.Cin * 2};
  int lower[2] = {-p.pad_l, -p.pad_t};
  int upper[2] = {pad_r - (k - 1), pad_b - (k - 1)};
  cuuint32_t estr[4] = {1, (cuuint32_t)p.stride, (cuuint32_t)p.stride, 1};
  CUresult r = enc(tm, (FRX_ENC_FP16 ? CU_TENSOR_MAP_DATA_TYPE_FLOAT16 : CU_TENSOR_MAP_DATA_TYPE_BFLOAT16), 4, const_cast<eh_t*>(p.A), dims, strides, lower, upper,
                   (cuuint32_t)TC_BK, (cuuint32_t)TC_BM, estr, CU_TENSOR_MAP_INTERLEAVE_NONE, CU_TENSOR_MAP_SWIZZLE_128B,
                   CU_TENSOR_MAP_L2_PROMOTION_L2_128B, CU_TENSOR_MAP_FLOAT_OOB_FILL_NONE);
  return r == CUDA_SUCCESS ? 0 : (int)cudaErrorInvalidValue;
}

template <int NCOLS>
static int tc_launch_ws(const TcGemmP& p_in, int num_sms, cudaStream_t st) {
  TcGemmP p = p_in;
  const size_t smem = (size_t)WS_STAGES * (TC_A_BYTES + (size_t)p.BN * TC_BK * 2) + 1024;
  static SmemOptIn opt, opt_gelu;
  {
    cudaError_t e = opt.ensure(tc_igemm_ws_kernel<NCOLS, false>, smem, true);
    if (e == cudaSuccess) e = opt_gelu.ensure(tc_igemm_ws_kernel<NCOLS, true>, smem, true);
    if (e != cudaSuccess) return (int)e;
  }
  const int tiles = ((p.M + TC_BM - 1) / TC_BM) * ((p.N + p.BN - 1) / p.BN);
  int per_sm = (int)((227 * 1024) / (smem + 2048));
  if (per_sm > 512 / NCOLS) per_sm = 512 / NCOLS;
  if (per_sm > 4) per_sm = 4;
  if (per_sm < 1) per_sm = 1;
  const int grid = tiles < num_sms * per_sm ? tiles : num_sms * per_sm;
  CUtensorMap tmA, tmW;
  int rc;
  p.im2col = 0;
  if (p.conv && p.Wpad && p.Cin <= TC_BK && p.M % (p.OH * p.OW) == 0 && make_tmap_im2col(&tmA, p) == 0) {
    p.im2col = 1;
    rc = make_tmap_2d(&tmW, p.Wpad, p.N, (long long)p.KW * p.KW * TC_BK, (long long)p.KW * p.KW * TC_BK, p.BN);
  } else {
    rc = make_tmap_2d(&tmW, p.W, p.N, p.K, p.ldw, p.BN);
    if (rc) return rc;
    if (!p.conv) rc = make_tmap_2d(&tmA, p.A, p.M, p.K, p.lda, TC_BM);
    else tmA = tmW;
  }
  if (rc) return rc;
  if (getenv("FRX_DEBUG"))
    fprintf(stderr, "[frx] tc gemm M=%d N=%d K=%d BN=%d conv=%d Cin=%d stride=%d -> %s, grid %d\n", p.M, p.N, p.K, p.BN, p.conv,
            p.Cin, p.stride, p.im2col ? "TMA im2col" : (p.conv ? "cp.async gather" : "TMA dense"), grid);
  if (p.act == ACT_GELU) tc_igemm_ws_kernel<NCOLS, true><<<grid, WS_THREADS, smem, st>>>(p, tmA, tmW);
  else tc_igemm_ws_kernel<NCOLS, false><<<grid, WS_THREADS, smem, st>>>(p, tmA, tmW);
  return 0;
}

int launch_tc_igemm_ws(TcGemmP p, int num_sms, cudaStream_t st) {
  if (p.BN == 0) {
    p.BN = tc_pick_bn(p.N);
    const int tiles_m = (p.M + TC_BM - 1) / TC_BM;
    while (p.BN > 64 && p.BN % 32 == 0 && p.N % (p.BN / 2) == 0 && tiles_m * ((p.N + p.BN - 1) / p.BN) < num_sms) p.BN /= 2;
  }
  if (p.BN <= 32) { p.BN = 32; return tc_launch_ws<64>(p, num_sms, st); }
  if (p.BN <= 64) return tc_launch_ws<128>(p, num_sms, st);
  if (p.BN <= 128) return tc_launch_ws<256>(p, num_sms, st);
  return tc_launch_ws<512>(p, num_sms, st);
}

int launch_tc_igemm(TcGemmP p, cudaStream_t st) {
  if (p.act == ACT_GELU) {
    int dev = 0, sms = 148;
    cudaGetDevice(&dev);
    cudaDeviceGetAttribute(&sms, cudaDevAttrMultiProcessorCount, dev);
    return launch_tc_igemm_ws(p, sms, st);
  }
  if (p.BN == 0) p.BN = tc_pick_bn(p.N);
  {
    const int kb = (p.K + TC_BK - 1) / TC_BK;
    const size_t stage = TC_A_BYTES + (size_t)p.BN * TC_BK * 2;
    p.stages = (kb > 3 && 3 * stage <= 72 * 1024) ? 3 : 2;
  }
  if (p.BN <= 32) { p.BN = 32; return tc_launch<32>(p, st); }
  if (p.BN <= 64) return tc_launch<64>(p, st);
  if (p.BN <= 128) return tc_launch<128>(p, st);
  return tc_launch<256>(p, st);
}

__global__ void __launch_bounds__(256) f32_to_h16_kernel(const float* __restrict__ in, eh_t* __restrict__ out, long long n) {
  long long i = ((long long)blockIdx.x * blockDim.x + threadIdx.x) * 4;
  if (i + 3 < n) {
    float4 v = __ldg(reinterpret_cast<const float4*>(in + i));
    *reinterpret_cast<uint2*>(out + i) = make_uint2(eh2_pack(v.x, v.y), eh2_pack(v.z, v.w));
  } else {
    for (; i < n; ++i) out[i] = eh_from_float(in[i]);
  }
}

void launch_f32_to_h16(const float* in, eh_t* out, long long n, cudaStream_t st) {
  f32_to_h16_kernel<<<(unsigned)((n / 4 + 256) / 256), 256, 0, st>>>(in, out, n);
}


__global__ void __launch_bounds__(256) h16_to_f32_kernel(const eh_t* __restrict__ in, float* __restrict__ out, long long n) {
  long long i = (long long)blockIdx.x * blockDim.x + threadIdx.x;
  if (i < n) out[i] = eh_to_float(in[i]);
}
void launch_h16_to_f32(const eh_t* in, float* out, long long n, cudaStream_t st) {
  h16_to_f32_kernel<<<(unsigned)((n + 255) / 256), 256, 0, st>>>(in, out, n);
}


__global__ void __launch_bounds__(256) pad_conv_weights_kernel(const eh_t* __restrict__ in, eh_t* __restrict__ out,
                                                               long long rows, int Cin) {
  long long i = (long long)blockIdx.x * blockDim.x + threadIdx.x;
  if (i >= rows * 64) return;
  const int ci = (int)(i & 63);
  out[i] = ci < Cin ? in[(i >> 6) * Cin + ci] : eh_from_float(0.f);
}
void launch_pad_conv_weights(const eh_t* in, eh_t* out, long long rows, int Cin, cudaStream_t st) {
  pad_conv_weights_kernel<<<(unsigned)((rows * 64 + 255) / 256), 256, 0, st>>>(in, out, rows, Cin);
}

}
```

### p4-fr-sorry-math-but-love-you_b200/csrc/runtime.cu

```cuda
#include <cmath>
#include <cstdarg>
#include <cstdio>
#include <cstring>
#include <map>
#include <string>
#include <vector>

#include "../../include/frx.h"
#include "kernels.h"
#include "runtime.h"

using namespace frx;

static int fail(frx_handle* h, const char* fmt, ...) {
  char buf[1024];
  va_list ap;
  va_start(ap, fmt);
  vsnprintf(buf, sizeof buf, fmt, ap);
  va_end(ap);
  if (h) h->err = buf;
  return 1;
}

#define CK(expr)                                                                          \
// ... 61 lines not shown
  const HostTensor* t = find(h, name);
  if (!t) return fail(h, "missing tensor '%s'", name.c_str());
  std::vector<int64_t> s(shape);
  if (t->shape != s) {
    std::string got, want;
    for (auto v : t->shape) got += std::to_string(v) + ",";
    for (auto v : s) want += std::to_string(v) + ",";
    return fail(h, "tensor '%s' has shape [%s] expected [%s]", name.c_str(), got.c_str(), want.c_str());
  }
  *out = t;
  return 0;
}

static int fold_bn(frx_handle* h, ArenaBuilder& ab, const std::string& p, int C, float eps,
                   const float* conv_bias, size_t* off_scale, size_t* off_shift) {
  const HostTensor *w, *b, *mu, *var;
  if (need(h, p + ".weight", {C}, &w) || need(h, p + ".bias", {C}, &b) ||
      need(h, p + ".running_mean", {C}, &mu) || need(h, p + ".running_var", {C}, &var))
    return 1;
  *off_scale = ab.add(nullptr, C);
  *off_shift = ab.add(nullptr, C);
  for (int c = 0; c < C; ++c) {
    float invstd = 1.0f / sqrtf(var->f[c] + eps);
    float alpha = w->f[c] * invstd;
    float beta = b->f[c] - mu->f[c] * alpha;
    if (conv_bias) beta += conv_bias[c] * alpha;
    ab.at(*off_scale)[c] = alpha;
    ab.at(*off_shift)[c] = beta;
  }
  return 0;
}

static int pack_conv(frx_handle* h, ArenaBuilder& ab, const std::string& name, int O, int I, int k,
                     size_t* off) {
  const HostTensor* w;
  if (need(h, name, {O, I, k, k}, &w)) return 1;
  *off = ab.add(nullptr, (size_t)O * I * k * k);
  float* d = ab.at(*off);
  for (int o = 0; o < O; ++o)
    for (int i = 0; i < I; ++i)
      for (int t = 0; t < k * k; ++t) d[((size_t)o * k * k + t) * I + i] = w->f[((size_t)o * I + i) * k * k + t];
  return 0;
}

static int pack_dw(frx_handle* h, ArenaBuilder& ab, const std::string& name, int C, size_t* off) {
  const HostTensor* w;
  if (need(h, name, {C, 1, 3, 3}, &w)) return 1;
  *off = ab.add(nullptr, (size_t)9 * C);
  float* d = ab.at(*off);
  for (int c = 0; c < C; ++c)
    for (int t = 0; t < 9; ++t) d[(size_t)t * C + c] = w->f[(size_t)c * 9 + t];
  return 0;
}

static void put_transposed(float* dst, int Ntot, int col0, const float* w, int N, int K) {
  for (int n = 0; n < N; ++n)
    for (int k = 0; k < K; ++k) dst[(size_t)k * Ntot + col0 + n] = w[(size_t)n * K + k];
}

static void same_pad(int in, int k, int stride, int* out, int* pad_lo) {
  *out = (in + stride - 1) / stride;
  if (stride == 1) { *pad_lo = (k - 1) / 2; return; }
  int pad = (*out - 1) * stride + k - in;
  if (pad < 0) pad = 0;
  *pad_lo = pad / 2;
}

static const int kArch[6][7] = {
    {0, 2, 3, 1, 1, 24, 0},  {1, 4, 3, 2, 4, 48, 0},    {1, 4, 3, 2, 4, 64, 0},
    {2, 6, 3, 2, 4, 128, 25}, {2, 9, 3, 1, 6, 160, 25}, {2, 15, 3, 2, 6, 256, 25}};

extern "C" const char* frx_version(void) { return "frx 0.1 sm_100a"; }

extern "C" const char* frx_last_error(const frx_handle* h) { return h ? h->err.c_str() : "null handle"; }

extern "C" int frx_create(const frx_config* cfg, frx_handle** out) {
  if (!cfg || !out) return 1;
  frx_handle* h = new frx_handle();
  h->cfg = *cfg;
  *out = h;
  int ndev = 0;
  cudaError_t e = cudaGetDeviceCount(&ndev);
  if (e != cudaSuccess || ndev == 0)
    return fail(h, "no CUDA device available (%s): frx has no CPU fallback", cudaGetErrorString(e));
  if (cfg->device < 0 || cfg->device >= ndev) return fail(h, "device %d out of range", cfg->device);
  ON_DEVICE(cfg->device);
  cudaDeviceProp prop;
  CK(cudaGetDeviceProperties(&prop, cfg->device));
  if (prop.major != 10) return fail(h, "device is sm_%d%d; frx is built for sm_100a (B200) only", prop.major, prop.minor);
  h->num_sms = prop.multiProcessorCount;
  if (cfg->network != FRX_NET_EFFICIENT_SATRN && cfg->network != FRX_NET_LITE_SATRN && cfg->network != FRX_NET_SWIN)
    return fail(h, "unknown network %d", cfg->network);
  if (cfg->network == FRX_NET_SWIN && (cfg->height != 384 || cfg->width != 384 || cfg->in_ch != 3 || cfg->enc_hidden != 1024))
    return fail(h, "SWIN is fixed to Swin-B/384: 384x384x3 input, 1024-wide memory (networks/SWIN.py:1028-1031)");
  if (cfg->dec_hidden % cfg->dec_heads || (cfg->dec_hidden / cfg->dec_heads != 32 && cfg->dec_hidden / cfg->dec_heads != 64))
    return fail(h, "decoder head_dim must be 32 or 64");
  if (cfg->dec_hidden > 512) return fail(h, "decoder hidden_dim > 512 not supported");
  if (cfg->max_batch <= 0 || cfg->max_steps <= 0) return fail(h, "max_batch/max_steps must be positive");
  return 0;
}

extern "C" void frx_destroy(frx_handle* h) {
  if (!h) return;
  DeviceGuard guard;
  guard.enter(h->cfg.device);
  frx_train_destroy(h);
  for (auto& kv : h->graphs) cudaGraphExecDestroy(kv.second.exec);
  for (void* p : h->allocs) cudaFree(p);
  for (auto& kv : h->taps) cudaFree(kv.second.data);
  if (h->ev[0]) for (int i = 0; i < 5; ++i) cudaEventDestroy(h->ev[i]);
  for (auto& sl : h->pipe) {
    if (sl.h2d) { cudaEventDestroy(sl.h2d); cudaEventDestroy(sl.enc); cudaEventDestroy(sl.done); cudaEventDestroy(sl.d2h); }
  }
  if (h->pipe_h2d) { cudaStreamDestroy(h->pipe_h2d); cudaStreamDestroy(h->pipe_d2h); cudaStreamDestroy(h->pipe_enc); }
  delete h;
}

extern "C" int frx_load_tensor(frx_handle* h, const char* name, const void* data, const int64_t* shape,
                               int32_t ndim, int32_t dtype) {
  if (!h || !name || !data) return fail(h, "frx_load_tensor: null argument");
  HostTensor t;
  size_t n = 1;
  for (int i = 0; i < ndim; ++i) { t.shape.push_back(shape[i]); n *= (size_t)shape[i]; }
  if (dtype == FRX_DTYPE_F32) {
    t.f.resize(n);
    CK(cudaMemcpy(t.f.data(), data, n * sizeof(float), cudaMemcpyDefault));
  } else if (dtype == FRX_DTYPE_I64) {
    std::vector<int64_t> tmp(n);
    CK(cudaMemcpy(tmp.data(), data, n * sizeof(int64_t), cudaMemcpyDefault));
    t.f.resize(n);
    for (size_t i = 0; i < n; ++i) t.f[i] = (float)tmp[i];
  } else {
    return fail(h, "frx_load_tensor('%s'): unsupported dtype %d", name, dtype);
  }
  h->raw[name] = std::move(t);
  h->finalized = false;
  return 0;
}

extern "C" int frx_set_option(frx_handle* h, const char* key, int64_t value) {
  if (!h || !key) return 1;
  ON_DEVICE(h->cfg.device);
  std::string k(key);
  if (k == "taps") h->opt_taps = value != 0;
  else if (k == "graphs") h->opt_graphs = value != 0;
  else if (k == "step16") h->opt_step16 = value != 0;
  else if (k == "pipe_enc") h->opt_pipe_enc = value != 0;
  else if (k == "timing") h->opt_timing = value != 0;
  else if (k == "cluster_images") {}
  else if (k == "dec_hpc") h->opt_dec_hpc = (value == 1 || value == 2) ? (int)value : 0;
  else if (k == "conv24") h->opt_conv24 = value != 0;
  else if (k == "enc_fp32") h->opt_enc_fp32 = value != 0;
  else if (k == "tc_ws") h->opt_tc_ws = value != 0;
  else if (k == "train_splitk") h->opt_train_splitk = value != 0;
  else if (k == "tc_im2col") h->opt_tc_im2col = value != 0;
  else if (k == "prof") {
    h->opt_prof = value != 0;
    if (h->opt_prof && !h->prof) { void* p; if (dev_alloc(h, &p, 16 * 8)) return 1; h->prof = (long long*)p; }
  }
  else if (k == "parts") {
    if (h->ws_ready && ((int)value & 3) != h->opt_parts)
      return fail(h, "option 'parts' cannot change after the first frx_finalize_weights (create a new handle)");
    h->opt_parts = (int)value & 3;
    h->finalized = false;
  }
  else return fail(h, "unknown option '%s'", key);
  return 0;
}

extern "C" int64_t frx_launch_count(const frx_handle* h) { return h ? h->launches : 0; }
extern "C" int64_t frx_device_bytes(const frx_handle* h) { return h ? h->device_bytes : 0; }

extern "C" int frx_read_prof(frx_handle* h, int64_t* out16) {
  if (!h || !out16 || !h->prof) return fail(h, "profiling not enabled (frx_set_option(h, \"prof\", 1))");
  ON_DEVICE(h->cfg.device);
  CK(cudaMemcpy(out16, h->prof, 16 * 8, cudaMemcpyDeviceToHost));
  return 0;
}

extern "C" int frx_last_timing(const frx_handle* h, float* ms4) {
  if (!h || !ms4) return 1;
  for (int i = 0; i < 4; ++i) ms4[i] = h->last_ms[i];
  return 0;
}

static int pack_trunk_efficientnet(frx_handle* h, ArenaBuilder& ab) {
  const frx_config& c = h->cfg;
  const std::string e = "encoder.shallow_cnn.";
  const HostTensor* w;
  if (need(h, e + "conv_stem.weight", {24, c.in_ch, 3, 3}, &w)) return 1;
  h->stem_w = ab.add(w->f.data(), w->f.size());
  if (fold_bn(h, ab, e + "bn1", 24, 1e-3f, nullptr, &h->stem_sc, &h->stem_sh)) return 1;
  int cin = 24;
  h->blocks.clear();
  for (int s = 0; s < 6; ++s) {
    for (int r = 0; r < kArch[s][1]; ++r) {
      BlockW b{};
      b.kind = kArch[s][0];
      b.k = kArch[s][2];
      b.stride = r == 0 ? kArch[s][3] : 1;
      b.cin = cin;
      b.cout = kArch[s][5];
      b.mid = cin * kArch[s][4];
      b.se_r = cin * kArch[s][6] / 100;
      b.residual = (b.cin == b.cout && b.stride == 1);
      std::string p = e + "eff_block." + std::to_string(s) + "." + std::to_string(r);
      b.name = "eff_block." + std::to_string(s) + "." + std::to_string(r);
      if (b.kind == 0) {
        if (pack_conv(h, ab, p + ".conv.weight", b.cout, b.cin, b.k, &b.w_a)) return 1;
        if (fold_bn(h, ab, p + ".bn1", b.cout, 1e-3f, nullptr, &b.sc_a, &b.sh_a)) return 1;
      } else if (b.kind == 1) {
        if (pack_conv(h, ab, p + ".conv_exp.weight", b.mid, b.cin, b.k, &b.w_a)) return 1;
        if (fold_bn(h, ab, p + ".bn1", b.mid, 1e-3f, nullptr, &b.sc_a, &b.sh_a)) return 1;
        if (pack_conv(h, ab, p + ".conv_pwl.weight", b.cout, b.mid, 1, &b.w_b)) return 1;
        if (fold_bn(h, ab, p + ".bn2", b.cout, 1e-3f, nullptr, &b.sc_b, &b.sh_b)) return 1;
      } else {
        if (pack_conv(h, ab, p + ".conv_pw.weight", b.mid, b.cin, 1, &b.w_a)) return 1;
        if (fold_bn(h, ab, p + ".bn1", b.mid, 1e-3f, nullptr, &b.sc_a, &b.sh_a)) return 1;
        if (pack_dw(h, ab, p + ".conv_dw.weight", b.mid, &b.w_dw)) return 1;
        if (fold_bn(h, ab, p + ".bn2", b.mid, 1e-3f, nullptr, &b.sc_dw, &b.sh_dw)) return 1;
        const HostTensor *w1, *b1, *w2, *b2;
        if (need(h, p + ".se.conv_reduce.weight", {b.se_r, b.mid, 1, 1}, &w1) ||
            need(h, p + ".se.conv_reduce.bias", {b.se_r}, &b1) ||
            need(h, p + ".se.conv_expand.weight", {b.mid, b.se_r, 1, 1}, &w2) ||
            need(h, p + ".se.conv_expand.bias", {b.mid}, &b2))
          return 1;
        b.se_w1 = ab.add(w1->f.data(), w1->f.size());
        b.se_b1 = ab.add(b1->f.data(), b1->f.size());
        b.se_w2 = ab.add(w2->f.data(), w2->f.size());
        b.se_w2t = ab.add(nullptr, w2->f.size());
        for (int cc = 0; cc < b.mid; ++cc)
          for (int rr = 0; rr < b.se_r; ++rr) ab.at(b.se_w2t)[(size_t)rr * b.mid + cc] = w2->f[(size_t)cc * b.se_r + rr];
        b.se_b2 = ab.add(b2->f.data(), b2->f.size());
        if (pack_conv(h, ab, p + ".conv_pwl.weight", b.cout, b.mid, 1, &b.w_b)) return 1;
        if (fold_bn(h, ab, p + ".bn3", b.cout, 1e-3f, nullptr, &b.sc_b, &b.sh_b)) return 1;
      }
      h->blocks.push_back(b);
      cin = b.cout;
    }
  }
  if (pack_conv(h, ab, e + "conv_last.weight", c.enc_hidden, 256, 1, &h->last_w)) return 1;
  if (fold_bn(h, ab, e + "bn2", c.enc_hidden, 1e-5f, nullptr, &h->last_sc, &h->last_sh)) return 1;
  return 0;
}

static int pack_trunk_lite(frx_handle* h, ArenaBuilder& ab) {
  const frx_config& c = h->cfg;
  const std::string e = "encoder.shallow_cnn.";
  int H = c.enc_hidden;
  int chans[4][2] = {{c.in_ch, H / 2}, {H / 2, H}, {H, H}, {H, H}};
  for (int i = 0; i < 4; ++i) {
    LiteConvW& L = h->lite[i];
    L.cin = chans[i][0];
    L.cout = chans[i][1];
    if (i == 0) {
      const HostTensor* w;
      if (need(h, e + "conv0.weight", {L.cout, L.cin, 3, 3}, &w)) return 1;
      L.w = ab.add(w->f.data(), w->f.size());
    } else if (pack_conv(h, ab, e + "conv" + std::to_string(i) + ".weight", L.cout, L.cin, 3, &L.w)) {
      return 1;
    }
    if (fold_bn(h, ab, e + "batch_norm" + std::to_string(i), L.cout, 1e-5f, nullptr, &L.sc, &L.sh)) return 1;
  }
  return 0;
}

static int pack_swin(frx_handle* h, ArenaBuilder& ab) {
  const std::string e = "encoder.";
  const int E = 128, R0 = 96, WS = 12;
  const int depths[4] = {2, 2, 18, 2}, heads[4] = {4, 8, 16, 32};
  auto vec = [&](const std::string& name, std::initializer_list<int64_t> shape, size_t* off) -> int {
    const HostTensor* t;
    if (need(h, name, shape, &t)) return 1;
    *off = ab.add(t->f.data(), t->f.size());
    return 0;
  };
  if (vec(e + "patch_embed.proj.weight", {E, 3, 4, 4}, &h->sw_pe_w) || vec(e + "patch_embed.proj.bias", {E}, &h->sw_pe_b) ||
      vec(e + "patch_embed.norm.weight", {E}, &h->sw_pe_g) || vec(e + "patch_embed.norm.bias", {E}, &h->sw_pe_beta) ||
      vec(e + "absolute_pos_embed", {1, R0 * R0, E}, &h->sw_ape) || vec(e + "norm.weight", {8 * E}, &h->sw_norm_g) ||
      vec(e + "norm.bias", {8 * E}, &h->sw_norm_b))
    return 1;
  h->sw_blocks.clear();
  h->sw_merges.clear();
  for (int i = 0; i < 4; ++i) {
    const int dim = E << i, res = R0 >> i;
    for (int j = 0; j < depths[i]; ++j) {
      SwinBlockW b{};
      b.dim = dim; b.res = res; b.heads = heads[i];
      b.ws = WS; b.shift = (j % 2 == 0) ? 0 : WS / 2;
      if (res <= WS) { b.ws = res; b.shift = 0; }
      const std::string p = e + "layers." + std::to_string(i) + ".blocks." + std::to_string(j) + ".";
      const int T = (2 * b.ws - 1) * (2 * b.ws - 1);
      if (vec(p + "norm1.weight", {dim}, &b.n1_g) || vec(p + "norm1.bias", {dim}, &b.n1_b) ||
          vec(p + "attn.relative_position_bias_table", {T, b.heads}, &b.bias_table) ||
          vec(p + "attn.qkv.weight", {3 * dim, dim}, &b.qkv_w) || vec(p + "attn.qkv.bias", {3 * dim}, &b.qkv_b) ||
          vec(p + "attn.proj.weight", {dim, dim}, &b.proj_w) || vec(p + "attn.proj.bias", {dim}, &b.proj_b) ||
          vec(p + "norm2.weight", {dim}, &b.n2_g) || vec(p + "norm2.bias", {dim}, &b.n2_b) ||
          vec(p + "mlp.fc1.weight", {4 * dim, dim}, &b.fc1_w) || vec(p + "mlp.fc1.bias", {4 * dim}, &b.fc1_b) ||
          vec(p + "mlp.fc2.weight", {dim, 4 * dim}, &b.fc2_w) || vec(p + "mlp.fc2.bias", {dim}, &b.fc2_b))
        return 1;
      h->sw_blocks.push_back(b);
    }
    if (i < 3) {
      SwinMergeW m{};
      m.dim = dim; m.res = res;
      const std::string p = e + "layers." + std::to_string(i) + ".downsample.";
// ... 278 lines not shown
  const float* gen = find(h, "decoder.generator.weight")->f.data();
  h->gen_wb = pack_bf16_copy(ab, h->gen_w, (size_t)V * D);
  for (int l = 0; l < L; ++l) {
    DecLayerW& Wl = h->dec[l];
    Wl.wb_o = pack_bf16_copy(ab, Wl.w_o, (size_t)D * D);
    Wl.wb_q2 = pack_bf16_copy(ab, Wl.w_q2, (size_t)D * D);
    Wl.wb_o2 = pack_bf16_copy(ab, Wl.w_o2, (size_t)D * D);
    Wl.wb_f0 = pack_bf16_copy(ab, Wl.w_f0, (size_t)F * D);
    Wl.wb_f1 = pack_bf16_copy(ab, Wl.w_f1, (size_t)D * F);
    Wl.wb_sqkv = pack_bf16_copy(ab, Wl.w_sqkv, (size_t)3 * D * D);
  }
  auto pack_geometry = [&](int CL, std::vector<DecPackW>& dp, size_t& first) {
    const int SW = D / CL, FS = F / CL, NTS = SW / 8, NTE = FS / 8, NG = 256 / CL / 8;
    dp.assign(L, DecPackW{});
    first = pack_frag_stage(ab, CL, 3 * NTS, D, [&](int r, int tile, int gid) {
      const char* names[3] = {"self_attention_layer.q_linear", "self_attention_layer.k_linear", "self_attention_layer.v_linear"};
      return W(0, names[tile / NTS]) + (size_t)(r * SW + (tile % NTS) * 8 + gid) * D;
    });
    for (int l = 0; l < L; ++l) {
      DecPackW& P = dp[l];
      auto square = [&](const char* name, int K) {
        const float* w = W(l, name);
        return pack_frag_stage(ab, CL, NTS, K, [=](int r, int tile, int gid) { return w + (size_t)(r * SW + tile * 8 + gid) * K; });
      };
      P.w_o = square("self_attention_layer.out_linear", D);
      P.w_q2 = square("attention_layer.q_linear", D);
      P.w_o2 = square("attention_layer.out_linear", D);
      P.w_f1 = square("feedforward_layer.linear1", F);
      const float* f0 = W(l, "feedforward_layer.linear0");
      P.w_f0 = pack_frag_stage(ab, CL, NTE, D, [=](int r, int tile, int gid) {
        return f0 + (size_t)(r * FS + tile * 8 + gid) * D;
      });
      const float* wk = W(l, "self_attention_layer.k_linear");
      const float* wv = W(l, "self_attention_layer.v_linear");
      if (l + 1 < L) {
        const float* nq = W(l + 1, "self_attention_layer.q_linear");
        const float* nk = W(l + 1, "self_attention_layer.k_linear");
        const float* nv = W(l + 1, "self_attention_layer.v_linear");
        P.w_next = pack_frag_stage(ab, CL, 5 * NTS, D, [=](int r, int tile, int gid) {
          const float* segs[5] = {wk, wv, nq, nk, nv};
          return segs[tile / NTS] + (size_t)(r * SW + (tile % NTS) * 8 + gid) * D;
        });
      } else {
        P.w_next = pack_frag_stage(ab, CL, 2 * NTS + NG, D, [=](int r, int tile, int gid) -> const float* {
          if (tile < 2 * NTS) return (tile < NTS ? wk : wv) + (size_t)(r * SW + (tile % NTS) * 8 + gid) * D;
          int n = r * (256 / CL) + (tile - 2 * NTS) * 8 + gid;
          return n < V ? gen + (size_t)n * D : nullptr;
        });
      }
    }
  };
  pack_geometry(c.dec_heads, h->dpack, h->dpack_first);
  if (D == 256) pack_geometry(c.dec_heads / 2, h->dpack2, h->dpack2_first);
  return 0;
}

extern "C" int frx_finalize_weights(frx_handle* h) {
  if (!h) return 1;
  const frx_config& c = h->cfg;
  ON_DEVICE(c.device);
  int down = c.network == FRX_NET_LITE_SATRN ? 16 : 32;
  h->feat_h = c.height / down;
  h->feat_w = c.width / down;
  ArenaBuilder ab;
  const bool want_enc = h->opt_parts & 1, want_dec = h->opt_parts & 2;
  if (want_enc) {
    if (c.network == FRX_NET_SWIN) {
      if (pack_swin(h, ab)) return 1;
    } else {
      if (c.network == FRX_NET_EFFICIENT_SATRN) {
        if (pack_trunk_efficientnet(h, ab)) return 1;
      } else if (pack_trunk_lite(h, ab)) {
        return 1;
      }
      if (pack_encoder(h, ab)) return 1;
    }
  }
  if (want_dec && pack_decoder(h, ab)) return 1;
  if (want_dec && c.precision == FRX_PREC_BF16 && pack_decoder_bf16(h, ab)) return 1;
  if (c.precision == FRX_PREC_BF16) {
    if (want_enc && c.network == FRX_NET_EFFICIENT_SATRN) pack_encoder_bf16(h, ab);
    if (want_enc && c.network == FRX_NET_LITE_SATRN) {
      for (int i = 1; i < 4; ++i) h->lite[i].wb = pack_bf16_copy(ab, h->lite[i].w, (size_t)h->lite[i].cout * 9 * h->lite[i].cin);
      pack_encoder_layers_bf16(h, ab);
    }
    if (want_enc && c.network == FRX_NET_SWIN) {
      for (SwinBlockW& b : h->sw_blocks) {
        const size_t C = b.dim;
        b.qkv_wb = pack_bf16_copy(ab, b.qkv_w, 3 * C * C);
        b.proj_wb = pack_bf16_copy(ab, b.proj_w, C * C);
        b.fc1_wb = pack_bf16_copy(ab, b.fc1_w, 4 * C * C);
        b.fc2_wb = pack_bf16_copy(ab, b.fc2_w, 4 * C * C);
      }
      for (SwinMergeW& m : h->sw_merges) m.red_wb = pack_bf16_copy(ab, m.red_w, (size_t)8 * m.dim * m.dim);
    }
    if (want_dec) h->cross_wb = pack_bf16_copy(ab, h->w_cross, (size_t)c.dec_layers * 2 * c.dec_hidden * c.dec_src);
  }
  size_t bytes = ab.host.size() * sizeof(float);
  if (h->arena) CK(cudaDeviceSynchronize());
  if (!h->arena || h->arena_bytes != bytes) {
    if (h->arena) {
      for (size_t i = 0; i < h->allocs.size(); ++i)
        if (h->allocs[i] == (void*)h->arena) { h->allocs.erase(h->allocs.begin() + i); break; }
      cudaFree(h->arena);
      h->device_bytes -= (int64_t)h->arena_bytes;
      h->arena = nullptr;
    }
    void* p;
    if (dev_alloc(h, &p, bytes)) return 1;
    h->arena = (float*)p;
    h->arena_bytes = bytes;
  }
  CK(cudaMemcpy(h->arena, ab.host.data(), bytes, cudaMemcpyHostToDevice));

  if (!h->ws_ready) {
    const size_t B = c.max_batch;
    size_t act_max = 0, mid_max = 0;
    if (c.network == FRX_NET_EFFICIENT_SATRN) {
      int H = (c.height - 3) / 2 + 1, W = (c.width - 3) / 2 + 1;
      act_max = (size_t)H * W * 24;
      for (const BlockW& b : h->blocks) {
        int OH, OW, pl;
        same_pad(H, b.k, b.stride, &OH, &pl);
        same_pad(W, b.k, b.stride, &OW, &pl);
        size_t mid = b.kind == 1 ? (size_t)OH * OW * b.mid : (b.kind == 2 ? (size_t)H * W * b.mid : 0);
        if (mid > mid_max) mid_max = mid;
        H = OH; W = OW;
        if ((size_t)H * W * b.cout > act_max) act_max = (size_t)H * W * b.cout;
      }
    } else {
      act_max = (size_t)c.height * c.width * (c.enc_hidden / 2);
      mid_max = act_max;
    }
    size_t S = (size_t)h->feat_h * h->feat_w, C = c.enc_hidden;
    size_t enc_act = S * 3 * C;
    if (enc_act > mid_max) mid_max = enc_act;
    if (S * C > act_max) act_max = S * C;
    void* p;
    if (want_enc && c.network == FRX_NET_SWIN) {
      const size_t tok = 96 * 96;
      for (int i = 0; i < 2; ++i) { if (dev_alloc(h, &p, B * tok * 128 * 4)) return 1; h->sw_x[i] = (float*)p; }
      if (dev_alloc(h, &p, B * tok * 128 * 4)) return 1; h->sw_a = (float*)p;
      if (dev_alloc(h, &p, B * tok * 384 * 4)) return 1; h->sw_qkv = (float*)p;
      if (dev_alloc(h, &p, B * tok * 512 * 4)) return 1; h->sw_hid = (float*)p;
      if (c.precision == FRX_PREC_BF16) {
        if (dev_alloc(h, &p, B * tok * 128 * 2)) return 1; h->sw_ab = p;
        if (dev_alloc(h, &p, B * tok * 512 * 2)) return 1; h->sw_hidb = p;
      }
    } else if (want_enc) {
      for (int i = 0; i < 2; ++i) { if (dev_alloc(h, &p, B * act_max * 4)) return 1; h->act[i] = (float*)p; }
      for (int i = 0; i < 2; ++i) { if (dev_alloc(h, &p, B * mid_max * 4)) return 1; h->mid[i] = (float*)p; }
      if (dev_alloc(h, &p, B * 2048 * 4 * 2)) return 1;
      h->gate = (float*)p;
    }
    const size_t D = c.dec_hidden, F = c.dec_filter, L = c.dec_layers, T = c.max_steps, V = c.num_classes;
    if (want_dec) {
    if (dev_alloc(h, &p, L * B * T * D * 4)) return 1; h->kself = (float*)p;
    if (dev_alloc(h, &p, L * B * T * D * 4)) return 1; h->vself = (float*)p;
    if (dev_alloc(h, &p, B * S * L * 2 * D * 4)) return 1; h->cross = (float*)p;
    float** small[] = {&h->dx, &h->datt, &h->dpre1, &h->dpre2, &h->du, &h->dw, &h->dq2};
    for (float** q : small) { if (dev_alloc(h, &p, B * D * 4)) return 1; *q = (float*)p; }
    if (dev_alloc(h, &p, B * 3 * D * 4)) return 1; h->dqkv = (float*)p;
    if (dev_alloc(h, &p, B * F * 4)) return 1; h->dff = (float*)p;
    if (dev_alloc(h, &p, B * T * V * 4)) return 1; h->logits_int = (float*)p;
    if (dev_alloc(h, &p, B * T * 8)) return 1; h->tokens_int = (long long*)p;
    if (dev_alloc(h, &p, B * T * 8)) return 1; h->forced_int = (long long*)p;
    if (dev_alloc(h, &p, B * 4)) return 1; h->cur_tok = (int*)p;
    if (c.precision == FRX_PREC_BF16) {
      if (dev_alloc(h, &p, L * B * T * D * 2)) return 1; h->kself_bf = p;
      if (dev_alloc(h, &p, L * B * T * D * 2)) return 1; h->vself_bf = p;
      if (dev_alloc(h, &p, L * B * S * D * 2)) return 1; h->kcross_bf = p;
      if (dev_alloc(h, &p, L * B * S * D * 2)) return 1; h->vcross_bf = p;
      if (dev_alloc(h, &p, B * S * (size_t)c.dec_src * 2)) return 1; h->mem_bf = p;
    }
    }
    if (dev_alloc(h, &p, B * S * C * 4)) return 1; h->memory_int = (float*)p;
    if (dev_alloc(h, &p, (size_t)c.in_ch * c.height * c.width * B * 4)) return 1; h->images_int = (float*)p;
    for (int i = 0; i < 5; ++i) CK(cudaEventCreate(&h->ev[i]));
    h->ws_ready = true;
  }
  for (auto& kv : h->graphs) cudaGraphExecDestroy(kv.second.exec);
  h->graphs.clear();
  h->finalized = true;
  return 0;
}

static int tap(frx_handle* h, const std::string& name, const float* src, int B, int H, int W, int C,
               cudaStream_t st) {
  if (!h->opt_taps) return 0;
  Tap& t = h->taps[name];
  size_t n = (size_t)B * H * W * C;
  if (t.capacity < n) {
    if (t.data) cudaFree(t.data);
    CK(cudaMalloc((void**)&t.data, n * 4));
    t.capacity = n;
  }
  t.shape[0] = B; t.shape[1] = H; t.shape[2] = W; t.shape[3] = C;
  CK(cudaMemcpyAsync(t.data, src, n * 4, cudaMemcpyDeviceToDevice, st));
  return 0;
}

extern "C" int frx_read_tap(frx_handle* h, const char* name, float* out, int64_t capacity, int64_t* count,
                            int32_t* shape4, void* stream) {
  if (!h || !name) return 1;
  auto it = h->taps.find(name);
  if (it == h->taps.end()) return fail(h, "no tap named '%s' (enable with frx_set_option(h,\"taps\",1))", name);
  const Tap& t = it->second;
  int64_t n = (int64_t)t.shape[0] * t.shape[1] * t.shape[2] * t.shape[3];
  if (count) *count = n;
  if (shape4) for (int i = 0; i < 4; ++i) shape4[i] = t.shape[i];
  if (out) {
    if (capacity < n) return fail(h, "tap '%s' needs %lld floats", name, (long long)n);
    CK(cudaMemcpyAsync(out, t.data, n * 4, cudaMemcpyDeviceToDevice, (cudaStream_t)stream));
  }
  return 0;
}

static int tap_bf16(frx_handle* h, const std::string& name, const void* src, int B, int H, int W, int C, cudaStream_t st) {
  if (!h->opt_taps) return 0;
  Tap& t = h->taps[name];
  size_t n = (size_t)B * H * W * C;
  if (t.capacity < n) {
    if (t.data) cudaFree(t.data);
    CK(cudaMalloc((void**)&t.data, n * 4));
    t.capacity = n;
  }
  t.shape[0] = B; t.shape[1] = H; t.shape[2] = W; t.shape[3] = C;
  launch_h16_to_f32((const eh_t*)src, t.data, (long long)n, st);
  CKL();
  return 0;
}

static GemmP dense_gemm(const float* A, int M, int K, const float* W, int N, float* C, int ldc) {
  GemmP g{};
  g.A = A; g.W = W; g.C = C; g.M = M; g.N = N; g.K = K; g.lda = K; g.ldc = ldc; g.conv = 0; g.rows_per_img = 1;
  return g;
}

static GemmP conv_gemm(const float* A, int B, int H, int W, int Cin, const float* Wt, int Cout, int k,
                       int stride, float* C, int* OH, int* OW) {
  GemmP g{};
  int pt, pl;
  same_pad(H, k, stride, OH, &pt);
  same_pad(W, k, stride, OW, &pl);
  g.A = A; g.W = Wt; g.C = C;
  g.M = B * (*OH) * (*OW); g.N = Cout; g.K = k * k * Cin; g.lda = 0; g.ldc = Cout;
  g.conv = 1; g.H = H; g.Wd = W; g.Cin = Cin; g.OH = *OH; g.OW = *OW; g.KH = k; g.KW = k;
  g.stride = stride; g.pad_t = pt; g.pad_l = pl; g.rows_per_img = 1;
  return g;
}

static int run_trunk_efficientnet(frx_handle* h, const float* images, int B, float** out, cudaStream_t st) {
  const frx_config& c = h->cfg;
  const float* A = h->arena;
  int H = (c.height - 3) / 2 + 1, W = (c.width - 3) / 2 + 1;
  float* x = h->act[0];
  float* y = h->act[1];
  launch_stem_conv(images, A + h->stem_w, A + h->stem_sc, A + h->stem_sh, x, B, c.in_ch, c.height, c.width, H, W, 24, st);
  CKL();
  if (tap(h, "stem", x, B, H, W, 24, st)) return 1;
  for (const BlockW& b : h->blocks) {
    int OH, OW;
    if (b.kind == 0) {
      GemmP g = conv_gemm(x, B, H, W, b.cin, A + b.w_a, b.cout, b.k, b.stride, y, &OH, &OW);
      g.scale = A + b.sc_a; g.shift = A + b.sh_a; g.act = ACT_SILU;
      if (b.residual) { g.res = x; g.ldr = b.cout; }
      launch_igemm_f32(g, st); CKL();
    } else if (b.kind == 1) {
      GemmP g = conv_gemm(x, B, H, W, b.cin, A + b.w_a, b.mid, b.k, b.stride, h->mid[0], &OH, &OW);
      g.scale = A + b.sc_a; g.shift = A + b.sh_a; g.act = ACT_SILU;
      launch_igemm_f32(g, st); CKL();
      GemmP g2 = dense_gemm(h->mid[0], B * OH * OW, b.mid, A + b.w_b, b.cout, y, b.cout);
      g2.scale = A + b.sc_b; g2.shift = A + b.sh_b; g2.act = ACT_NONE;
      if (b.residual) { g2.res = x; g2.ldr = b.cout; }
      launch_igemm_f32(g2, st); CKL();
    } else {
      GemmP g = dense_gemm(x, B * H * W, b.cin, A + b.w_a, b.mid, h->mid[0], b.mid);
      g.scale = A + b.sc_a; g.shift = A + b.sh_a; g.act = ACT_SILU;
      launch_igemm_f32(g, st); CKL();
      int pt, pl;
      same_pad(H, b.k, b.stride, &OH, &pt);
      same_pad(W, b.k, b.stride, &OW, &pl);
      DwP d{h->mid[0], A + b.w_dw, A + b.sc_dw, A + b.sh_dw, h->mid[1], B, H, W, b.mid, OH, OW, b.stride, pt, pl, ACT_SILU};
      launch_dwconv_f32(d, st); CKL();
      launch_se_gate_f32(h->mid[1], A + b.se_w1, A + b.se_b1, A + b.se_w2, A + b.se_b2, h->gate, B, OH * OW, b.mid, b.se_r, st);
      CKL();
      GemmP g2 = dense_gemm(h->mid[1], B * OH * OW, b.mid, A + b.w_b, b.cout, y, b.cout);
      g2.gate = h->gate; g2.rows_per_img = OH * OW;
      g2.scale = A + b.sc_b; g2.shift = A + b.sh_b; g2.act = ACT_NONE;
      if (b.residual) { g2.res = x; g2.ldr = b.cout; }
      launch_igemm_f32(g2, st); CKL();
    }
    H = OH; W = OW;
    float* t = x; x = y; y = t;
    if (tap(h, b.name, x, B, H, W, b.cout, st)) return 1;
  }
  GemmP g = dense_gemm(x, B * H * W, 256, A + h->last_w, c.enc_hidden, y, c.enc_hidden);
  g.scale = A + h->last_sc; g.shift = A + h->last_sh; g.act = ACT_SILU;
  launch_igemm_f32(g, st); CKL();
  if (H != h->feat_h || W != h->feat_w) return fail(h, "trunk output %dx%d != expected %dx%d", H, W, h->feat_h, h->feat_w);
  *out = y;
  return 0;
}

static TcGemmP tc_dense(const void* A, int M, int K, const float* arena, size_t w_off, int N, void* C, int out_f32) {
  TcGemmP g{};
  g.A = (const eh_t*)A; g.W = (const eh_t*)(arena + w_off); g.C = C;
  g.M = M; g.N = N; g.K = K; g.lda = K; g.ldw = K; g.ldc = N; g.out_f32 = out_f32;
  return g;
}

static TcGemmP tc_conv(const void* A, int B, int H, int W, int Cin, const float* arena, size_t w_off, int Cout, int k,
                       int stride, void* C, int* OH, int* OW) {
  TcGemmP g{};
  int pt, pl;
  same_pad(H, k, stride, OH, &pt);
  same_pad(W, k, stride, OW, &pl);
  g.A = (const eh_t*)A; g.W = (const eh_t*)(arena + w_off); g.C = C;
  g.M = B * (*OH) * (*OW); g.N = Cout; g.K = k * k * Cin; g.ldw = g.K; g.ldc = Cout;
  g.conv = 1; g.H = H; g.Wd = W; g.Cin = Cin; g.OH = *OH; g.OW = *OW; g.KW = k; g.stride = stride; g.pad_t = pt; g.pad_l = pl;
  return g;
}

#define TCL(g)                                                                                         \
  do {                                                                                                 \
    int rc__ = h->opt_tc_ws ? launch_tc_igemm_ws(g, h->num_sms, st) : launch_tc_igemm(g, st);          \
    if (rc__) return fail(h, "tcgen05 GEMM configuration failed: %s", cudaGetErrorString((cudaError_t)rc__)); \
    CKL();                                                                                             \
  } while (0)

static int encoder_layers_16(frx_handle* h, float* tf, float* xf, eh_t* m0, eh_t* m1, int B, float* memory, cudaStream_t st) {
  typedef eh_t bf;
  const frx_config& c = h->cfg;
  const float* A = h->arena;
  const int fh = h->feat_h, fw = h->feat_w, S = fh * fw, C = c.enc_hidden, F = c.enc_filter, M = B * S;
  float* other = tf;
  for (int i = 0; i < c.enc_layers; ++i) {
    const EncLayerW& L = h->enc[i];
    launch_layernorm_bf16out(xf, nullptr, A + L.ln_g, A + L.ln_b, m0, M, C, 0, st); CKL();
    float* qkv = (float*)m1;
    TcGemmP g = tc_dense(m0, M, C, A, L.wb_qkv, 3 * C, qkv, 1);
    g.shift = A + L.b_qkv;
    TCL(g);
    if (!launch_enc_attn_mma_bf16(qkv, m0, B, S, C, c.enc_heads, st)) launch_enc_attn_bf16out(qkv, m0, B, S, C, c.enc_heads, st);
    CKL();
    float* proj = (float*)m1;
    TcGemmP go = tc_dense(m0, M, C, A, L.wb_o, C, proj, 1);
    go.shift = A + L.b_o;
    TCL(go);
    launch_layernorm_bf16out(proj, xf, A + L.ln_g, A + L.ln_b, m0, M, C, S, st); CKL();
    TcGemmP g0 = tc_dense(m0, M, C, A, L.wb_c0, F, m1, 0);
    g0.scale = A + L.sc_c0; g0.shift = A + L.sh_c0; g0.act = ACT_RELU;
    TCL(g0);
    launch_dwconv_bf16(m1, A + L.w_dw, A + L.sc_dw, A + L.sh_dw, m0, B, fh, fw, F, fh, fw, 1, 1, 1, ACT_RELU, st); CKL();
    float* dst = (i == c.enc_layers - 1) ? memory : other;
    TcGemmP g1 = tc_dense(m0, M, F, A, L.wb_c1, C, dst, 1);
    g1.scale = A + L.sc_c1; g1.shift = A + L.sh_c1; g1.act = ACT_RELU; g1.res = xf; g1.res_f32 = 1; g1.ldr = C;
    TCL(g1);
    if (tap(h, "enc_layer" + std::to_string(i), dst, B, fh, fw, C, st)) return 1;
    other = xf;
    xf = dst;
  }
  return 0;
}


static int encode_bf16(frx_handle* h, const float* images, int B, float* memory, cudaStream_t st) {
  const frx_config& c = h->cfg;
  const float* A = h->arena;
  typedef eh_t bf;
  int H = (c.height - 3) / 2 + 1, W = (c.width - 3) / 2 + 1;
  bf* x = (bf*)h->act[0];
  bf* y = (bf*)h->act[1];
  bf* m0 = (bf*)h->mid[0];
  bf* m1 = (bf*)h->mid[1];
  launch_stem_conv_bf16(images, A + h->stem_w, A + h->stem_sc, A + h->stem_sh, x, B, c.in_ch, c.height, c.width, H, W, 24, st);
  CKL();
  if (tap_bf16(h, "stem", x, B, H, W, 24, st)) return 1;
  for (const BlockW& b : h->blocks) {
    int OH, OW;
    if (b.kind == 0 && b.w_frag24 && h->opt_conv24) {
      OH = H; OW = W;
      launch_conv3x3_c24_bf16(x, A + b.w_frag24, A + b.sc_a, A + b.sh_a, y, B, H, W, b.residual ? 1 : 0, st);
      CKL();
    } else if (b.kind == 0) {
      TcGemmP g = tc_conv(x, B, H, W, b.cin, A, b.wb_a, b.cout, b.k, b.stride, y, &OH, &OW);
      if (b.wb_a_pad && h->opt_tc_im2col) g.Wpad = (const eh_t*)(A + b.wb_a_pad);
      g.scale = A + b.sc_a; g.shift = A + b.sh_a; g.act = ACT_SILU;
      if (b.residual) { g.res = x; g.ldr = b.cout; }
      TCL(g);
    } else if (b.kind == 1) {
      TcGemmP g = tc_conv(x, B, H, W, b.cin, A, b.wb_a, b.mid, b.k, b.stride, m0, &OH, &OW);
      if (b.wb_a_pad && h->opt_tc_im2col) g.Wpad = (const eh_t*)(A + b.wb_a_pad);
      g.scale = A + b.sc_a; g.shift = A + b.sh_a; g.act = ACT_SILU;
      TCL(g);
      TcGemmP g2 = tc_dense(m0, B * OH * OW, b.mid, A, b.wb_b, b.cout, y, 0);
      g2.scale = A + b.sc_b; g2.shift = A + b.sh_b;
      if (b.residual) { g2.res = x; g2.ldr = b.cout; }
      TCL(g2);
    } else {
      TcGemmP g = tc_dense(x, B * H * W, b.cin, A, b.wb_a, b.mid, m0, 0);
      g.scale = A + b.sc_a; g.shift = A + b.sh_a; g.act = ACT_SILU;
      TCL(g);
      int pt, pl;
      same_pad(H, b.k, b.stride, &OH, &pt);
      same_pad(W, b.k, b.stride, &OW, &pl);
      launch_mbconv_dw_se_bf16(m0, A + b.w_dw, A + b.sc_dw, A + b.sh_dw, m1, h->gate, h->gate + (size_t)B * 2048,
                               A + b.se_w1, A + b.se_b1, A + b.se_w2t, A + b.se_b2, B, H, W, b.mid, OH, OW, b.stride, pt, pl,
                               b.se_r, st);
      CKL(); h->launches += 2;
      TcGemmP g2 = tc_dense(m1, B * OH * OW, b.mid, A, b.wb_b, b.cout, y, 0);
      g2.scale = A + b.sc_b; g2.shift = A + b.sh_b;
      if (b.residual) { g2.res = x; g2.ldr = b.cout; }
      TCL(g2);
    }
    H = OH; W = OW;
    bf* t = x; x = y; y = t;
    if (tap_bf16(h, b.name, x, B, H, W, b.cout, st)) return 1;
  }
  if (H != h->feat_h || W != h->feat_w) return fail(h, "trunk output %dx%d != expected %dx%d", H, W, h->feat_h, h->feat_w);
  const int fh = h->feat_h, fw = h->feat_w, S = fh * fw, C = c.enc_hidden, F = c.enc_filter, M = B * S;
  float* tf = (float*)y;
  {
    TcGemmP g = tc_dense(x, M, 256, A, h->last_wb, C, tf, 1);
    g.scale = A + h->last_sc; g.shift = A + h->last_sh; g.act = ACT_SILU;
    TCL(g);
  }
  if (tap(h, "trunk", tf, B, fh, fw, C, st)) return 1;
  float* xf = (float*)x;
  launch_pe2d_f32(tf, A + h->pe_w0, A + h->pe_b0, A + h->pe_w1, A + h->pe_b1, A + h->pe_h, A + h->pe_w, xf, B, fh, fw, C, st);
  CKL();
  if (tap(h, "pe2d", xf, B, fh, fw, C, st)) return 1;
  return encoder_layers_16(h, tf, xf, m0, m1, B, memory, st);
}

static int encode_swin(frx_handle* h, const float* images, int B, float* memory, cudaStream_t st) {
  const float* A = h->arena;
  float* x = h->sw_x[0];
  float* y = h->sw_x[1];
  launch_swin_patch_embed(images, A + h->sw_pe_w, A + h->sw_pe_b, A + h->sw_pe_g, A + h->sw_pe_beta, A + h->sw_ape, x, B, 384,
                          96, 128, st);
  CKL();
  if (tap(h, "embed", x, B, 96, 96, 128, st)) return 1;
  size_t bi = 0;
  const int depths[4] = {2, 2, 18, 2};
  for (int i = 0; i < 4; ++i) {
    for (int j = 0; j < depths[i]; ++j, ++bi) {
      const SwinBlockW& b = h->sw_blocks[bi];
      const int M = B * b.res * b.res, C = b.dim;
      if (h->cfg.precision == FRX_PREC_BF16) {
        eh_t* ab16 = (eh_t*)h->sw_ab;
        launch_layernorm_bf16out(x, nullptr, A + b.n1_g, A + b.n1_b, ab16, M, C, 0, st); CKL();
        { TcGemmP g = tc_dense(ab16, M, C, A, b.qkv_wb, 3 * C, h->sw_qkv, 1); g.shift = A + b.qkv_b; TCL(g); }
        if (!launch_swin_window_attn_mma(h->sw_qkv, A + b.bias_table, ab16, B, b.res, C, b.heads, b.ws, b.shift, st)) {
          launch_swin_window_attn(h->sw_qkv, A + b.bias_table, h->sw_a, B, b.res, C, b.heads, b.ws, b.shift, st); CKL();
          launch_f32_to_h16(h->sw_a, ab16, (long long)M * C, st);
        }
        CKL();
        { TcGemmP g = tc_dense(ab16, M, C, A, b.proj_wb, C, y, 1); g.shift = A + b.proj_b; g.res = x; g.res_f32 = 1; g.ldr = C; TCL(g); }
        launch_layernorm_bf16out(y, nullptr, A + b.n2_g, A + b.n2_b, ab16, M, C, 0, st); CKL();
        { TcGemmP g = tc_dense(ab16, M, C, A, b.fc1_wb, 4 * C, h->sw_hidb, 0); g.shift = A + b.fc1_b; g.act = ACT_GELU; TCL(g); }
        { TcGemmP g = tc_dense(h->sw_hidb, M, 4 * C, A, b.fc2_wb, C, x, 1); g.shift = A + b.fc2_b; g.res = y; g.res_f32 = 1; g.ldr = C; TCL(g); }
        if (tap(h, "block" + std::to_string(i) + "." + std::to_string(j), x, B, b.res, b.res, C, st)) return 1;
        continue;
      }
      launch_layernorm_f32(x, nullptr, A + b.n1_g, A + b.n1_b, h->sw_a, M, C, 0, st); CKL();
      GemmP g = dense_gemm(h->sw_a, M, C, A + b.qkv_w, 3 * C, h->sw_qkv, 3 * C);
      g.shift = A + b.qkv_b;
      launch_igemm_f32(g, st); CKL();
      launch_swin_window_attn(h->sw_qkv, A + b.bias_table, h->sw_a, B, b.res, C, b.heads, b.ws, b.shift, st); CKL();
      GemmP gp = dense_gemm(h->sw_a, M, C, A + b.proj_w, C, y, C);
      gp.shift = A + b.proj_b; gp.res = x; gp.ldr = C;
      launch_igemm_f32(gp, st); CKL();
      launch_layernorm_f32(y, nullptr, A + b.n2_g, A + b.n2_b, h->sw_a, M, C, 0, st); CKL();
      GemmP g1 = dense_gemm(h->sw_a, M, C, A + b.fc1_w, 4 * C, h->sw_hid, 4 * C);
      g1.shift = A + b.fc1_b; g1.act = ACT_GELU;
      launch_igemm_f32(g1, st); CKL();
      GemmP g2 = dense_gemm(h->sw_hid, M, 4 * C, A + b.fc2_w, C, x, C);
      g2.shift = A + b.fc2_b; g2.res = y; g2.ldr = C;
      launch_igemm_f32(g2, st); CKL();
      if (tap(h, "block" + std::to_string(i) + "." + std::to_string(j), x, B, b.res, b.res, C, st)) return 1;
    }
    if (i < 3) {
      const SwinMergeW& m = h->sw_merges[i];
      const int M2 = B * (m.res / 2) * (m.res / 2);
      launch_swin_patch_merge(x, h->sw_hid, B, m.res, m.dim, st); CKL();
      if (h->cfg.precision == FRX_PREC_BF16) {
        launch_layernorm_bf16out(h->sw_hid, nullptr, A + m.n_g, A + m.n_b, (eh_t*)h->sw_hidb, M2, 4 * m.dim, 0, st); CKL();
        TcGemmP g = tc_dense(h->sw_hidb, M2, 4 * m.dim, A, m.red_wb, 2 * m.dim, x, 1);
        TCL(g);
        if (tap(h, "merge" + std::to_string(i), x, B, m.res / 2, m.res / 2, 2 * m.dim, st)) return 1;
        continue;
      }
      launch_layernorm_f32(h->sw_hid, nullptr, A + m.n_g, A + m.n_b, h->sw_qkv, M2, 4 * m.dim, 0, st); CKL();
      GemmP g = dense_gemm(h->sw_qkv, M2, 4 * m.dim, A + m.red_w, 2 * m.dim, x, 2 * m.dim);
      launch_igemm_f32(g, st); CKL();
      if (tap(h, "merge" + std::to_string(i), x, B, m.res / 2, m.res / 2, 2 * m.dim, st)) return 1;
    }
  }
  launch_layernorm_f32(x, nullptr, A + h->sw_norm_g, A + h->sw_norm_b, memory, B * 144, 1024, 0, st); CKL();
  return 0;
}

static int run_trunk_lite(frx_handle* h, const float* images, int B, float** out, cudaStream_t st) {
  const frx_config& c = h->cfg;
  const float* A = h->arena;
  int H = c.height, W = c.width;
  float* x = h->act[0];
  float* y = h->act[1];
  if (c.precision == FRX_PREC_BF16 && !h->opt_enc_fp32 && h->lite[1].wb) {
    typedef eh_t bf;
    bf* xb = (bf*)h->act[0];
    bf* yb = (bf*)h->act[1];
    const LiteConvW& L0 = h->lite[0];
    launch_lite_conv0_pool_bf16(images, A + L0.w, A + L0.sc, A + L0.sh, yb, B, L0.cin, H, W, L0.cout, st); CKL();
    H /= 2; W /= 2;
    for (int i = 1; i < 4; ++i) {
      const LiteConvW& L = h->lite[i];
      int OH, OW;
      TcGemmP g = tc_conv(yb, B, H, W, L.cin, A, L.wb, L.cout, 3, 1, xb, &OH, &OW);
      g.scale = A + L.sc; g.shift = A + L.sh; g.act = ACT_RELU;
      TCL(g);
      const bool last = i == 3;
      float* f32_out = last ? h->act[1] + (size_t)B * (H / 2) * (W / 2) * L.cout : nullptr;
      launch_maxpool2_bf16(xb, yb, f32_out, B, H, W, L.cout, st); CKL();
      H /= 2; W /= 2;
      if (last) y = f32_out;
    }
    if (H != h->feat_h || W != h->feat_w) return fail(h, "trunk output %dx%d != expected %dx%d", H, W, h->feat_h, h->feat_w);
    if (tap(h, "lite_conv3", y, B, H, W, h->lite[3].cout, st)) return 1;
    *out = y;
    return 0;
  }
  for (int i = 0; i < 4; ++i) {
    const LiteConvW& L = h->lite[i];
    if (i == 0) {
      launch_direct_conv3x3(images, A + L.w, A + L.sc, A + L.sh, x, B, L.cin, H, W, H, W, L.cout, 1, 1, ACT_RELU, st);
      CKL();
    } else {
      int OH, OW;
      GemmP g = conv_gemm(y, B, H, W, L.cin, A + L.w, L.cout, 3, 1, x, &OH, &OW);
      g.scale = A + L.sc; g.shift = A + L.sh; g.act = ACT_RELU;
      launch_igemm_f32(g, st); CKL();
    }
    launch_maxpool2_f32(x, y, B, H, W, L.cout, st); CKL();
    H /= 2; W /= 2;
    if (tap(h, "lite_conv" + std::to_string(i), y, B, H, W, L.cout, st)) return 1;
  }
  if (H != h->feat_h || W != h->feat_w) return fail(h, "trunk output %dx%d != expected %dx%d", H, W, h->feat_h, h->feat_w);
  *out = y;
  return 0;
}

extern "C" int frx_encode(frx_handle* h, const float* images, int32_t B, float* memory, void* stream) {
  if (!h) return 1;
  if (!h->finalized) return fail(h, "frx_encode: weights not finalized");
  if (!(h->opt_parts & 1)) return fail(h, "frx_encode: handle was created without the encoder part");
  if (B <= 0 || B > h->cfg.max_batch) return fail(h, "frx_encode: batch %d outside (0, %d]", B, h->cfg.max_batch);
  const frx_config& c = h->cfg;
  cudaStream_t st = (cudaStream_t)stream;
  ON_DEVICE(c.device);
  if (c.network == FRX_NET_SWIN) return encode_swin(h, images, B, memory, st);
  if (c.precision == FRX_PREC_BF16 && !h->opt_enc_fp32 && c.network == FRX_NET_EFFICIENT_SATRN)
    return encode_bf16(h, images, B, memory, st);
  const float* A = h->arena;
// ... 706 lines not shown
```

### p4-fr-sorry-math-but-love-you_b200/csrc/runtime.h

```cpp
#pragma once
#include <cuda_runtime.h>
#include <stdint.h>

#include <map>
#include <string>
#include <tuple>
#include <vector>

#include "../../include/frx.h"

struct HostTensor {
  std::vector<int64_t> shape;
  std::vector<float> f;
};

struct BlockW {
  int kind;
  int cin, cout, k, stride, mid, se_r;
  bool residual;
  std::string name;
  size_t w_a, sc_a, sh_a;
  size_t w_dw, sc_dw, sh_dw;
  size_t se_w1, se_b1, se_w2, se_b2, se_w2t = 0;
  size_t w_b, sc_b, sh_b;
  size_t wb_a = 0, wb_b = 0;
  size_t wb_a_pad = 0;
  size_t w_frag24 = 0;
};
struct LiteConvW { int cin, cout; size_t w, sc, sh; size_t wb = 0; };
struct EncLayerW {
  size_t ln_g, ln_b, w_qkv, b_qkv, w_o, b_o;
  size_t w_c0, sc_c0, sh_c0, w_dw, sc_dw, sh_dw, w_c1, sc_c1, sh_c1;
  size_t wb_qkv = 0, wb_o = 0, wb_c0 = 0, wb_c1 = 0;
};
struct DecLayerW {
  size_t wt_o, b_o, wt_q2, b_q2, wt_o2, b_o2, wt_f0, b_f0, wt_f1, b_f1;
  size_t w_o, w_q2, w_o2, w_f0, w_f1, w_sqkv, b_sqkv;
  size_t wb_o = 0, wb_q2 = 0, wb_o2 = 0, wb_f0 = 0, wb_f1 = 0, wb_sqkv = 0;
  size_t ln1_g, ln1_b, ln2_g, ln2_b, ln3_g, ln3_b;
};
struct FusedW { size_t wt, b; int N; };
struct SwinBlockW {
  int dim, res, heads, ws, shift;
  size_t n1_g, n1_b, bias_table, qkv_w, qkv_b, proj_w, proj_b, n2_g, n2_b, fc1_w, fc1_b, fc2_w, fc2_b;
  size_t qkv_wb = 0, proj_wb = 0, fc1_wb = 0, fc2_wb = 0;
};
struct SwinMergeW { int dim, res; size_t red_w, n_g, n_b; size_t red_wb = 0; };
struct DecPackW { size_t w_o, w_q2, w_o2, w_f0, w_f1, w_next; };
struct Tap { float* data = nullptr; size_t capacity = 0; int shape[4] = {0, 0, 0, 0}; };
typedef std::tuple<int, int, int> GraphKey;
struct GraphEntry { cudaGraphExec_t exec; int64_t nodes; int64_t last_use = 0; };
constexpr size_t FRX_MAX_GRAPHS = 4;

struct BeamWs {
  double *hscore = nullptr, *nlogp = nullptr;
  int *hnode = nullptr, *nprev = nullptr, *ntok = nullptr, *nlen = nullptr, *nkv = nullptr, *chain = nullptr, *small = nullptr;
  float* logits = nullptr;
  int* host_flag = nullptr;
};
struct TfWs {
  float *x = nullptr, *y = nullptr, *z = nullptr, *qkv = nullptr, *ff = nullptr;
  unsigned char* mask = nullptr;
  void *xb = nullptr, *ffb = nullptr;
};

struct frx_handle {
  frx_config cfg{};
  std::string err;
  int num_sms = 0;
  std::map<std::string, HostTensor> raw;
  bool finalized = false, ws_ready = false;
  bool opt_taps = false, opt_graphs = true, opt_timing = false, opt_step16 = true, opt_pipe_enc = true;
  int* step_hist = nullptr;
  bool opt_prof = false;
  bool opt_tc_im2col = true;
  void* hook_wpad = nullptr; size_t hook_wpad_bytes = 0;
  bool opt_tc_ws = true;
  int opt_dec_hpc = 0;
  bool opt_conv24 = true;
  bool opt_enc_fp32 = false;
  long long* prof = nullptr;
  int opt_parts = 3;
  int feat_h = 0, feat_w = 0;
  std::vector<void*> allocs;
  int64_t device_bytes = 0, launches = 0;

  float* arena = nullptr;
  size_t arena_bytes = 0;
  size_t stem_w = 0, stem_sc = 0, stem_sh = 0, last_w = 0, last_sc = 0, last_sh = 0;
  std::vector<BlockW> blocks;
  LiteConvW lite[4]{};
  size_t pe_w0 = 0, pe_b0 = 0, pe_w1 = 0, pe_b1 = 0, pe_h = 0, pe_w = 0;
  std::vector<EncLayerW> enc;
  size_t sw_pe_w = 0, sw_pe_b = 0, sw_pe_g = 0, sw_pe_beta = 0, sw_ape = 0, sw_norm_g = 0, sw_norm_b = 0;
  std::vector<SwinBlockW> sw_blocks;
  std::vector<SwinMergeW> sw_merges;
  float *sw_x[2] = {nullptr, nullptr}, *sw_a = nullptr, *sw_qkv = nullptr, *sw_hid = nullptr;
  size_t emb = 0, pe1d = 0, gen_w = 0, gen_b = 0, w_cross = 0, b_cross = 0;
  size_t gen_wb = 0;
  size_t last_wb = 0, cross_wb = 0;
  std::vector<DecLayerW> dec;
  std::vector<FusedW> fused;
  std::vector<DecPackW> dpack;
  size_t dpack_first = 0;
  std::vector<DecPackW> dpack2;
  size_t dpack2_first = 0;

  float *act[2] = {nullptr, nullptr}, *mid[2] = {nullptr, nullptr}, *gate = nullptr;
  float *kself = nullptr, *vself = nullptr, *cross = nullptr;
  float *dx = nullptr, *dqkv = nullptr, *datt = nullptr, *dpre1 = nullptr, *dpre2 = nullptr, *du = nullptr,
        *dw = nullptr, *dq2 = nullptr, *dff = nullptr;
  float *logits_int = nullptr, *memory_int = nullptr, *images_int = nullptr;
  long long *tokens_int = nullptr, *forced_int = nullptr;
  int* cur_tok = nullptr;
  void* mem_bf = nullptr;
  void *kself_bf = nullptr, *vself_bf = nullptr, *kcross_bf = nullptr, *vcross_bf = nullptr;

  std::map<GraphKey, GraphEntry> graphs;
  int64_t graph_clock = 0;
  std::map<std::string, Tap> taps;
  cudaEvent_t ev[5] = {nullptr, nullptr, nullptr, nullptr, nullptr};
  struct PipeSlot {
    float *img = nullptr, *mem = nullptr;
    long long* tok = nullptr;
    cudaEvent_t h2d = nullptr, enc = nullptr, done = nullptr, d2h = nullptr;
    bool busy = false;
  };
  PipeSlot pipe[2];
  cudaStream_t pipe_h2d = nullptr, pipe_d2h = nullptr, pipe_enc = nullptr;
  float last_ms[4] = {0, 0, 0, 0};
  BeamWs beam;
  TfWs tf;
  int step_idx = 0, step_batch = 0;
  int *sift_flags = nullptr, *sift_limit = nullptr;
  int4* sift_state = nullptr;
  int sift_ids[6] = {0, 0, 0, 0, 0, 0};
  bool have_rules = false;
  bool timed_kernel = false;
  bool opt_train_splitk = true;
  bool dec_cluster_ok = false;
  void* train = nullptr;
  void *sw_ab = nullptr, *sw_hidb = nullptr;
};
```

Measured before the change: 13040.

## Fuse SE gate FC into dwconv tail and SE scaling into projection GEMM

The MBConv squeeze-excitation path used three launches: the depthwise conv plus mean, a separate SE FC kernel, and an elementwise apply kernel that rescaled the whole bf16 activation. Now the last-arriving CTA per image (counted with an atomic arrivals counter) computes the SE gate at the end of the depthwise kernel. The warp-specialized tcgen05 GEMM gains gate warps that multiply the A tile in shared memory by the per-image gate before the MMA consumes it. This removes two launches and a full read and write of the activation, at the cost of an extra barrier stage in the GEMM pipeline and fewer epilogue warps.

```diff
diff --git a/p4-fr-sorry-math-but-love-you_b200/csrc/common.cuh b/p4-fr-sorry-math-but-love-you_b200/csrc/common.cuh
--- a/p4-fr-sorry-math-but-love-you_b200/csrc/common.cuh
+++ b/p4-fr-sorry-math-but-love-you_b200/csrc/common.cuh
@@ -66,6 +66,22 @@
 __device__ __forceinline__ float eh_to_float(eh_t v) { return __bfloat162float(v); }
 __device__ __forceinline__ float2 eh2_unpack(uint32_t w) { return make_float2(__uint_as_float(w << 16), __uint_as_float(w & 0xffff0000u)); }
 #endif
+
+__device__ __forceinline__ void eh_unpack8(const uint4& u, float (&f)[8]) {
+  const uint32_t w[4] = {u.x, u.y, u.z, u.w};
+#pragma unroll
+  for (int i = 0; i < 4; ++i) {
+    const float2 t = eh2_unpack(w[i]);
+    f[2 * i] = t.x;
+    f[2 * i + 1] = t.y;
+  }
+}
+__device__ __forceinline__ uint4 eh_pack8(const float (&f)[8]) {
+  uint32_t w[4];
+#pragma unroll
+  for (int i = 0; i < 4; ++i) w[i] = eh2_pack(f[2 * i], f[2 * i + 1]);
+  return make_uint4(w[0], w[1], w[2], w[3]);
+}
 
 __device__ __forceinline__ float warp_sum(float v) {
 #pragma unroll
@@ -182,6 +198,8 @@
   int act;
   const void* res;
   int res_f32, ldr, out_f32;
+  const float* gate;
+  int rows_per_img;
 };
 
 struct SiftIds { int sos, eos, empty, lbrace, rbrace, underbar; };
diff --git a/p4-fr-sorry-math-but-love-you_b200/csrc/kernels.h b/p4-fr-sorry-math-but-love-you_b200/csrc/kernels.h
--- a/p4-fr-sorry-math-but-love-you_b200/csrc/kernels.h
+++ b/p4-fr-sorry-math-but-love-you_b200/csrc/kernels.h
@@ -62,10 +62,10 @@
                         int pad_l, int act, cudaStream_t st);
 void launch_se_scale_bf16(eh_t* x, const float* w1, const float* b1, const float* w2, const float* b2,
                           int B, int HW, int C, int R, cudaStream_t st);
-void launch_mbconv_dw_se_bf16(const eh_t* in, const float* w, const float* scale, const float* shift,
-                              eh_t* out, float* mean, float* gate, const float* w1, const float* b1,
-                              const float* w2, const float* b2, int B, int H, int W, int C, int OH, int OW, int stride,
-                              int pad_t, int pad_l, int R, cudaStream_t st);
+int launch_mbconv_dw_se_bf16(const eh_t* in, const float* w, const float* scale, const float* shift,
+                             eh_t* out, float* mean, float* gate, const float* w1, const float* b1,
+                             const float* w2, const float* b2, int B, int H, int W, int C, int OH, int OW, int stride,
+                             int pad_t, int pad_l, int R, int* arrivals, cudaStream_t st);
 void launch_layernorm_bf16out(const float* x, const float* res, const float* gamma, const float* beta,
                               eh_t* out, int M, int C, int scramble_S, cudaStream_t st);
 void launch_enc_attn_bf16out(const float* qkv, eh_t* out, int B, int S, int D, int heads, cudaStream_t st);
diff --git a/p4-fr-sorry-math-but-love-you_b200/csrc/kernels_bf16.cu b/p4-fr-sorry-math-but-love-you_b200/csrc/kernels_bf16.cu
--- a/p4-fr-sorry-math-but-love-you_b200/csrc/kernels_bf16.cu
+++ b/p4-fr-sorry-math-but-love-you_b200/csrc/kernels_bf16.cu
@@ -8,24 +8,6 @@
 #endif
 
 namespace frx {
-
-namespace {
-__device__ __forceinline__ void unpack8(const uint4& u, float (&f)[8]) {
-  const uint32_t w[4] = {u.x, u.y, u.z, u.w};
-#pragma unroll
-  for (int i = 0; i < 4; ++i) {
-    const float2 t = eh2_unpack(w[i]);
-    f[2 * i] = t.x;
-    f[2 * i + 1] = t.y;
-  }
-}
-__device__ __forceinline__ uint4 pack8(const float (&f)[8]) {
-  uint32_t w[4];
-#pragma unroll
-  for (int i = 0; i < 4; ++i) w[i] = eh2_pack(f[2 * i], f[2 * i + 1]);
-  return make_uint4(w[0], w[1], w[2], w[3]);
-}
-}
 
 __global__ void __launch_bounds__(256) stem_conv_bf16_kernel(const float* __restrict__ in, const float* __restrict__ w,
                                                              const float* __restrict__ scale, const float* __restrict__ shift,
@@ -64,7 +46,7 @@
   float o[8];
 #pragma unroll
   for (int j = 0; j < 8; ++j) o[j] = act_apply(acc[j] * ssc[co0 + j] + ssh[co0 + j], ACT_SILU);
-  *reinterpret_cast<uint4*>(out + pix * Cout + co0) = pack8(o);
+  *reinterpret_cast<uint4*>(out + pix * Cout + co0) = eh_pack8(o);
 }
 
 template <int COUT>
@@ -114,7 +96,7 @@
     float o[8];
 #pragma unroll
     for (int j = 0; j < 8; ++j) o[j] = act_apply(acc[g * 8 + j] * ssc[g * 8 + j] + ssh[g * 8 + j], ACT_SILU);
-    stage[threadIdx.x * (COUT / 8) + g] = pack8(o);
+    stage[threadIdx.x * (COUT / 8) + g] = eh_pack8(o);
   }
   __syncthreads();
   const long long cta_vecs = min((long long)blockDim.x, npix - pix0) * (COUT / 8);
@@ -158,7 +140,7 @@
       const int iw = ow * stride - pad_l + kw;
       if (iw < 0 || iw >= W) continue;
       float x[8];
-      unpack8(__ldg(reinterpret_cast<const uint4*>(in + (((long long)n * H + ih) * W + iw) * C + c)), x);
+      eh_unpack8(__ldg(reinterpret_cast<const uint4*>(in + (((long long)n * H + ih) * W + iw) * C + c)), x);
       const float4 w0 = __ldg(reinterpret_cast<const float4*>(w + (kh * 3 + kw) * C + c));
       const float4 w1 = __ldg(reinterpret_cast<const float4*>(w + (kh * 3 + kw) * C + c + 4));
       acc[0] = fmaf(x[0], w0.x, acc[0]); acc[1] = fmaf(x[1], w0.y, acc[1]);
@@ -170,7 +152,7 @@
   float o[8];
 #pragma unroll
   for (int j = 0; j < 8; ++j) o[j] = act_apply(acc[j] * __ldg(scale + c + j) + __ldg(shift + c + j), act);
-  *reinterpret_cast<uint4*>(out + pix * C + c) = pack8(o);
+  *reinterpret_cast<uint4*>(out + pix * C + c) = eh_pack8(o);
 }
 
 void launch_dwconv_bf16(const eh_t* in, const float* w, const float* scale, const float* shift,
@@ -197,7 +179,7 @@
     for (int j = 0; j < 8; ++j) s[j] = 0.f;
     for (int q = 0; q < HW; ++q) {
       float v[8];
-      unpack8(*reinterpret_cast<const uint4*>(xp + (long long)q * C + c8 * 8), v);
+      eh_unpack8(*reinterpret_cast<const uint4*>(xp + (long long)q * C + c8 * 8), v);
 #pragma unroll
       for (int j = 0; j < 8; ++j) s[j] += v[j];
     }
@@ -224,10 +206,10 @@
     const int c8 = i % (C / 8);
     uint4* ptr = reinterpret_cast<uint4*>(xp + (long long)(i / (C / 8)) * C + c8 * 8);
     float v[8];
-    unpack8(*ptr, v);
+    eh_unpack8(*ptr, v);
 #pragma unroll
     for (int j = 0; j < 8; ++j) v[j] *= gate[c8 * 8 + j];
-    *ptr = pack8(v);
+    *ptr = eh_pack8(v);
   }
 }
 
@@ -295,7 +277,7 @@
           const int iw = ow * stride - pad_l + kw;
           if (ih >= 0 && ih < H && iw >= 0 && iw < W) {
             float x[8], wv[8];
-            unpack8(tile[(ih * W + iw) * 8 + cg], x);
+            eh_unpack8(tile[(ih * W + iw) * 8 + cg], x);
             ld8s(kh * 3 + kw, wv);
 #pragma unroll
             for (int j = 0; j < 8; ++j) acc[j] = fmaf(x[j], wv[j], acc[j]);
@@ -308,10 +290,10 @@
         const float v = fmaf(acc[j], sc[j], sh[j]);
         o[j] = __fdividef(v, 1.f + __expf(-v));
       }
-      const uint4 packed = pack8(o);
+      const uint4 packed = eh_pack8(o);
       *reinterpret_cast<uint4*>(op + (long long)px * C + c) = packed;
       float back[8];
-      unpack8(packed, back);
+      eh_unpack8(packed, back);
 #pragma unroll
       for (int j = 0; j < 8; ++j) sum[j] += back[j];
     }
@@ -324,6 +306,75 @@
 #pragma unroll
     for (int i = 0; i < 32; ++i) s += red[i][threadIdx.x];
     mean[(long long)n * C + c0 + threadIdx.x] = s / (float)(OH * OW);
+  }
+}
+
+__device__ __forceinline__ void se_gate_tail(const float* mean, const float* __restrict__ w1, const float* __restrict__ b1,
+                                             const float* __restrict__ w2t, const float* __restrict__ b2,
+                                             float* __restrict__ gate, int* __restrict__ arrivals, int n, int C, int R,
+                                             float* smem) {
+  __shared__ int last;
+  __threadfence();
+  __syncthreads();
+  if (threadIdx.x == 0) {
+    last = atomicAdd(arrivals + n, 1) == (int)gridDim.x - 1;
+    if (last) arrivals[n] = 0;
+  }
+  __syncthreads();
+  if (!last) return;
+  __threadfence();
+  float* mv = smem;
+  float* red = smem + C;
+  const float* mp = mean + (long long)n * C;
+  for (int i = threadIdx.x; i < C; i += blockDim.x) {
+    float v;
+    asm volatile("ld.global.cg.f32 %0, [%1];\n" : "=f"(v) : "l"(mp + i));
+    mv[i] = v;
+  }
+  __syncthreads();
+  constexpr int ROWS = 2, CHN = 4;
+  const int warp = threadIdx.x >> 5, lane = threadIdx.x & 31, nwarps = blockDim.x >> 5;
+  for (int r0 = warp * ROWS; r0 < R; r0 += nwarps * ROWS) {
+    float s[ROWS] = {};
+#pragma unroll 3
+    for (int c4 = lane; c4 < C / 4; c4 += 32) {
+      const float4 m4 = *reinterpret_cast<const float4*>(mv + c4 * 4);
+#pragma unroll
+      for (int j = 0; j < ROWS; ++j) {
+        if (r0 + j < R) {
+          const float4 wv = __ldg(reinterpret_cast<const float4*>(w1 + (long long)(r0 + j) * C) + c4);
+          s[j] = fmaf(wv.x, m4.x, fmaf(wv.y, m4.y, fmaf(wv.z, m4.z, fmaf(wv.w, m4.w, s[j]))));
+        }
+      }
+    }
+#pragma unroll
+    for (int j = 0; j < ROWS; ++j) {
+      const float t = warp_sum(s[j]);
+      if (lane == 0 && r0 + j < R) red[r0 + j] = act_apply(t + __ldg(b1 + r0 + j), ACT_SILU);
+    }
+  }
+  __syncthreads();
+  for (int c0 = threadIdx.x; c0 < C; c0 += CHN * blockDim.x) {
+    float s[CHN];
+#pragma unroll
+    for (int j = 0; j < CHN; ++j) {
+      const int c = c0 + j * blockDim.x;
+      s[j] = c < C ? __ldg(b2 + c) : 0.f;
+    }
+#pragma unroll 2
+    for (int r = 0; r < R; ++r) {
+      const float hr = red[r];
+#pragma unroll
+      for (int j = 0; j < CHN; ++j) {
+        const int c = c0 + j * blockDim.x;
+        if (c < C) s[j] = fmaf(__ldg(w2t + (long long)r * C + c), hr, s[j]);
+      }
+    }
+#pragma unroll
+    for (int j = 0; j < CHN; ++j) {
+      const int c = c0 + j * blockDim.x;
+      if (c < C) gate[(long long)n * C + c] = 1.f / (1.f + expf(-s[j]));
+    }
   }
 }
 
@@ -333,7 +384,9 @@
                                                                  eh_t* __restrict__ out, float* __restrict__ mean,
                                                                  int H, int W, int C, int OH, int OW, int stride, int pad_t,
                                                                  int pad_l, const float* __restrict__ se_w1,
-                                                                 const float* __restrict__ se_w2, int se_floats) {
+                                                                 const float* __restrict__ se_w2, int se_floats,
+                                                                 const float* __restrict__ se_b1, const float* __restrict__ se_b2,
+                                                                 float* __restrict__ gate, int* __restrict__ arrivals, int R) {
   constexpr int NT = CH * 4, G8 = CH / 8, G4 = CH / 4;
   extern __shared__ __align__(16) unsigned char dw_smem[];
   {
@@ -345,7 +398,7 @@
   }
   uint4* tile = reinterpret_cast<uint4*>(dw_smem);
   float (*red)[CH + 1] = reinterpret_cast<float (*)[CH + 1]>(dw_smem + (size_t)H * W * G8 * 16);
-  const int n = blockIdx.x, c0 = blockIdx.y * CH;
+  const int n = blockIdx.y, c0 = blockIdx.x * CH;
   const eh_t* ip = in + (long long)n * H * W * C;
   for (int i = threadIdx.x; i < H * W * G8; i += NT) {
     const int px = i / G8, g = i - px * G8;
@@ -355,7 +408,7 @@
       v = __ldg(reinterpret_cast<const uint4*>(ip + (long long)px * C + c0 + g * 8));
 #else
       float x[8];
-      unpack8(__ldg(reinterpret_cast<const uint4*>(ip + (long long)px * C + c0 + g * 8)), x);
+      eh_unpack8(__ldg(reinterpret_cast<const uint4*>(ip + (long long)px * C + c0 + g * 8)), x);
       const __half2 h0 = __floats2half2_rn(x[0], x[1]), h1 = __floats2half2_rn(x[2], x[3]);
       const __half2 h2 = __floats2half2_rn(x[4], x[5]), h3 = __floats2half2_rn(x[6], x[7]);
       v = make_uint4(*reinterpret_cast<const uint32_t*>(&h0), *reinterpret_cast<const uint32_t*>(&h1),
@@ -481,6 +534,7 @@
     for (int i = 0; i < 16; ++i) s2 += red[i][threadIdx.x];
     mean[(long long)n * C + c0 + threadIdx.x] = s2 / (float)(OH * OW);
   }
+  if (gate) se_gate_tail(mean, se_w1, se_b1, se_w2, se_b2, gate, arrivals, n, C, R, reinterpret_cast<float*>(dw_smem));
 }
 
 constexpr int SE_IMGS = 4;
@@ -555,35 +609,39 @@
   const long long n = i / ((long long)C8 * HW);
   uint4* ptr = reinterpret_cast<uint4*>(x) + i;
   float v[8];
-  unpack8(*ptr, v);
+  eh_unpack8(*ptr, v);
   const float4 g0 = __ldg(reinterpret_cast<const float4*>(gate + n * C + c));
   const float4 g1 = __ldg(reinterpret_cast<const float4*>(gate + n * C + c + 4));
   v[0] *= g0.x; v[1] *= g0.y; v[2] *= g0.z; v[3] *= g0.w;
   v[4] *= g1.x; v[5] *= g1.y; v[6] *= g1.z; v[7] *= g1.w;
-  *ptr = pack8(v);
-}
-
-void launch_mbconv_dw_se_bf16(const eh_t* in, const float* w, const float* scale, const float* shift,
-                              eh_t* out, float* mean, float* gate, const float* w1, const float* b1,
-                              const float* w2, const float* b2, int B, int H, int W, int C, int OH, int OW, int stride,
-                              int pad_t, int pad_l, int R, cudaStream_t st) {
+  *ptr = eh_pack8(v);
+}
+
+int launch_mbconv_dw_se_bf16(const eh_t* in, const float* w, const float* scale, const float* shift,
+                             eh_t* out, float* mean, float* gate, const float* w1, const float* b1,
+                             const float* w2, const float* b2, int B, int H, int W, int C, int OH, int OW, int stride,
+                             int pad_t, int pad_l, int R, int* arrivals, cudaStream_t st) {
   dim3 g(B, (C + 63) / 64);
   const size_t smem = (size_t)H * W * 8 * 16 + 32 * 65 * sizeof(float) + 11 * 64 * sizeof(float);
   static SmemOptIn opt;
   opt.ensure(dwconv_se_mean_kernel, smem);
   if (C % 8 == 0) {
     constexpr int CH = 32;
-    const size_t sm4 = (size_t)H * W * (CH / 8) * 16 + 16 * (CH + 1) * sizeof(float);
+    size_t sm4 = (size_t)H * W * (CH / 8) * 16 + 16 * (CH + 1) * sizeof(float);
+    if (arrivals && sm4 < (size_t)(C + R) * sizeof(float)) sm4 = (size_t)(C + R) * sizeof(float);
     static SmemOptIn opt4;
     opt4.ensure(dwconv4_se_mean_kernel<CH>, sm4);
-    dwconv4_se_mean_kernel<CH><<<dim3(B, (C + CH - 1) / CH), CH * 4, sm4, st>>>(in, w, scale, shift, out, mean, H, W, C, OH, OW,
-                                                                             stride, pad_t, pad_l, w1, w2, R * C);
+    dwconv4_se_mean_kernel<CH><<<dim3((C + CH - 1) / CH, B), CH * 4, sm4, st>>>(
+        in, w, scale, shift, out, mean, H, W, C, OH, OW, stride, pad_t, pad_l, w1, w2, R * C, b1, b2,
+        arrivals ? gate : nullptr, arrivals, R);
+    if (arrivals) return 1;
   } else {
     dwconv_se_mean_kernel<<<g, 256, smem, st>>>(in, w, scale, shift, out, mean, H, W, C, OH, OW, stride, pad_t, pad_l, w1, w2, R * C);
   }
   se_fc_kernel<<<dim3((B + SE_IMGS - 1) / SE_IMGS, 2), 512, SE_IMGS * (C + R) * sizeof(float), st>>>(mean, w1, b1, w2, b2, gate, B, C, R);
   long long total8 = (long long)B * OH * OW * (C / 8);
   se_apply_kernel<<<(unsigned)((total8 + 255) / 256), 256, 0, st>>>(out, gate, total8, OH * OW, C);
+  return 3;
 }
 
 __device__ __forceinline__ uint32_t pack2(float lo, float hi) {
@@ -822,7 +880,7 @@
     const float m = fmaxf(fmaxf(fmaf(acc[0][j], s, t), fmaf(acc[1][j], s, t)), fmaxf(fmaf(acc[2][j], s, t), fmaf(acc[3][j], s, t)));
     o[j] = fmaxf(m, 0.f);
   }
-  *reinterpret_cast<uint4*>(out + pix * Cout + co0) = pack8(o);
+  *reinterpret_cast<uint4*>(out + pix * Cout + co0) = eh_pack8(o);
 }
 
 template <int KS, int Cout>
@@ -914,10 +972,10 @@
   const int ow = (int)(pix % OW), oh = (int)((pix / OW) % OH), n = (int)(pix / ((long long)OW * OH));
   const eh_t* base = in + (((long long)n * H + oh * 2) * W + ow * 2) * C + c;
   float a[8], b[8], d[8], e[8], o[8];
-  unpack8(__ldg(reinterpret_cast<const uint4*>(base)), a);
-  unpack8(__ldg(reinterpret_cast<const uint4*>(base + C)), b);
-  unpack8(__ldg(reinterpret_cast<const uint4*>(base + (long long)W * C)), d);
-  unpack8(__ldg(reinterpret_cast<const uint4*>(base + (long long)W * C + C)), e);
+  eh_unpack8(__ldg(reinterpret_cast<const uint4*>(base)), a);
+  eh_unpack8(__ldg(reinterpret_cast<const uint4*>(base + C)), b);
+  eh_unpack8(__ldg(reinterpret_cast<const uint4*>(base + (long long)W * C)), d);
+  eh_unpack8(__ldg(reinterpret_cast<const uint4*>(base + (long long)W * C + C)), e);
 #pragma unroll
   for (int j = 0; j < 8; ++j) o[j] = fmaxf(fmaxf(a[j], b[j]), fmaxf(d[j], e[j]));
   if (out_f32) {
@@ -925,7 +983,7 @@
     op[0] = make_float4(o[0], o[1], o[2], o[3]);
     op[1] = make_float4(o[4], o[5], o[6], o[7]);
   } else {
-    *reinterpret_cast<uint4*>(out + pix * C + c) = pack8(o);
+    *reinterpret_cast<uint4*>(out + pix * C + c) = eh_pack8(o);
   }
 }
 
diff --git a/p4-fr-sorry-math-but-love-you_b200/csrc/kernels_tc.cu b/p4-fr-sorry-math-but-love-you_b200/csrc/kernels_tc.cu
--- a/p4-fr-sorry-math-but-love-you_b200/csrc/kernels_tc.cu
+++ b/p4-fr-sorry-math-but-love-you_b200/csrc/kernels_tc.cu
@@ -409,13 +409,20 @@
 constexpr int WS_THREADS = (WS_TMA_WARP + 1) * 32;
 constexpr int WS_PROD_THREADS = WS_PROD_WARPS * 32;
 constexpr int WS_ROWS_PER_PASS = WS_PROD_THREADS / 8;
+#ifndef FRX_WS_GATE_WARPS
+#define FRX_WS_GATE_WARPS 4
+#endif
+constexpr int WS_GATE_WARPS = FRX_WS_GATE_WARPS;
+constexpr int WS_GATE_THREADS = WS_GATE_WARPS * 32;
+constexpr int WS_GATE_CHUNKS = TC_A_BYTES / 16 / WS_GATE_THREADS;
+static_assert(WS_GATE_WARPS % 4 == 0 && WS_GATE_WARPS <= WS_PROD_WARPS, "epilogue warps must cover whole TMEM lane quarters");
 constexpr int WS_A_PASSES = TC_BM / WS_ROWS_PER_PASS;
 
-template <int NCOLS, bool GELU>
+template <int NCOLS, bool GELU, bool GATE>
 __global__ void __launch_bounds__(WS_THREADS, NCOLS >= 256 ? 1 : 2) tc_igemm_ws_kernel(const TcGemmP p, const __grid_constant__ CUtensorMap tmA,
                                                                   const __grid_constant__ CUtensorMap tmW) {
   extern __shared__ unsigned char dyn_smem[];
-  __shared__ __align__(8) uint64_t full_bar[WS_STAGES], empty_bar[WS_STAGES], acc_full[2], acc_empty[2];
+  __shared__ __align__(8) uint64_t full_bar[WS_STAGES], empty_bar[WS_STAGES], gated_bar[WS_STAGES], acc_full[2], acc_empty[2];
   __shared__ uint32_t tmem_base_s;
 
   const int tid = threadIdx.x, warp = tid >> 5, lane = tid & 31;
@@ -427,6 +434,7 @@
   const int tiles_m = (p.M + TC_BM - 1) / TC_BM;
   const int num_tiles = tiles_m * tiles_n;
   const bool gather = p.conv && !p.im2col;
+  constexpr bool gated = GATE;
 
   if (warp == WS_MMA_WARP) {
     asm volatile("tcgen05.alloc.cta_group::1.sync.aligned.shared::cta.b32 [%0], %1;\n" ::"r"(smem_u32(&tmem_base_s)), "n"(NCOLS) : "memory");
@@ -434,9 +442,13 @@
   }
   if (tid == 0) {
 #pragma unroll
-    for (int s = 0; s < WS_STAGES; ++s) { mbar_init(&full_bar[s], (gather ? WS_PROD_THREADS : 0) + 1); mbar_init(&empty_bar[s], 1); }
+    for (int s = 0; s < WS_STAGES; ++s) {
+      mbar_init(&full_bar[s], (gather ? WS_PROD_THREADS : 0) + 1);
+      mbar_init(&empty_bar[s], 1);
+      mbar_init(&gated_bar[s], WS_GATE_THREADS);
+    }
     mbar_init(&acc_full[0], 1); mbar_init(&acc_full[1], 1);
-    const int epi_threads = (WS_EPI_WARPS + (gather ? 0 : WS_PROD_WARPS)) * 32;
+    const int epi_threads = gated ? (WS_MMA_WARP - WS_GATE_WARPS) * 32 : (WS_EPI_WARPS + (gather ? 0 : WS_PROD_WARPS)) * 32;
     mbar_init(&acc_empty[0], epi_threads); mbar_init(&acc_empty[1], epi_threads);
     asm volatile("fence.mbarrier_init.release.cluster;\n" ::: "memory");
   }
@@ -528,6 +540,39 @@
       for (int j = (it >= WS_LAG ? it - WS_LAG : 0); j < it; ++j) mbar_arrive(&full_bar[j % WS_STAGES]);
     }
     }
+  } else if (gated && warp < WS_GATE_WARPS) {
+    int it = 0;
+    for (int tile = blockIdx.x; tile < num_tiles; tile += gridDim.x) {
+      const int m0 = (tile / tiles_n) * TC_BM;
+      const float* grow[WS_GATE_CHUNKS];
+#pragma unroll
+      for (int i = 0; i < WS_GATE_CHUNKS; ++i) {
+        const int m = m0 + ((tid + WS_GATE_THREADS * i) >> 3);
+        grow[i] = m < p.M ? p.gate + (size_t)(m / p.rows_per_img) * p.K : nullptr;
+      }
+      for (int kb = 0; kb < KB; ++kb, ++it) {
+        const int stage = it % WS_STAGES;
+        mbar_wait(&full_bar[stage], (uint32_t)((it / WS_STAGES) & 1));
+        unsigned char* sa = dyn_smem + (smem0 - smem_u32(dyn_smem)) + (size_t)stage * stage_bytes;
+#pragma unroll
+        for (int i = 0; i < WS_GATE_CHUNKS; ++i) {
+          const int q = tid + WS_GATE_THREADS * i, row = q >> 3;
+          const int k = kb * TC_BK + (((q & 7) ^ (row & 7)) << 3);
+          if (grow[i] && k < p.K) {
+            uint4* ptr = reinterpret_cast<uint4*>(sa) + q;
+            float v[8];
+            eh_unpack8(*ptr, v);
+            const float4 g0 = __ldg(reinterpret_cast<const float4*>(grow[i] + k));
+            const float4 g1 = __ldg(reinterpret_cast<const float4*>(grow[i] + k + 4));
+            v[0] *= g0.x; v[1] *= g0.y; v[2] *= g0.z; v[3] *= g0.w;
+            v[4] *= g1.x; v[5] *= g1.y; v[6] *= g1.z; v[7] *= g1.w;
+            *ptr = eh_pack8(v);
+          }
+        }
+        asm volatile("fence.proxy.async.shared::cta;\n" ::: "memory");
+        mbar_arrive(&gated_bar[stage]);
+      }
+    }
   } else if (warp == WS_MMA_WARP) {
     if (lane == 0) {
       const uint32_t idesc = make_idesc(BN);
@@ -539,7 +584,7 @@
         const uint32_t tacc = tmem + (uint32_t)(a * (NCOLS / 2));
         for (int kb = 0; kb < KB; ++kb, ++it) {
           const int stage = it % WS_STAGES;
-          mbar_wait(&full_bar[stage], (uint32_t)((it / WS_STAGES) & 1));
+          mbar_wait(gated ? &gated_bar[stage] : &full_bar[stage], (uint32_t)((it / WS_STAGES) & 1));
           tc_fence_after();
           const uint32_t sa = smem0 + (uint32_t)stage * stage_bytes;
           const uint64_t adesc = make_smem_desc(sa), bdesc = make_smem_desc(sa + TC_A_BYTES);
@@ -553,8 +598,8 @@
     }
   } else if (warp < WS_MMA_WARP) {
     const int q = warp & 3;
-    const int nsub = (WS_EPI_WARPS + (gather ? 0 : WS_PROD_WARPS)) / 4;
-    const int sub = (gather ? warp - WS_PROD_WARPS : warp) >> 2;
+    const int nsub = gated ? (WS_MMA_WARP - WS_GATE_WARPS) / 4 : (WS_EPI_WARPS + (gather ? 0 : WS_PROD_WARPS)) / 4;
+    const int sub = (gated ? warp - WS_GATE_WARPS : (gather ? warp - WS_PROD_WARPS : warp)) >> 2;
     int ti = 0;
     for (int tile = blockIdx.x; tile < num_tiles; tile += gridDim.x, ++ti) {
       const int a = ti & 1;
@@ -658,10 +703,11 @@
 static int tc_launch_ws(const TcGemmP& p_in, int num_sms, cudaStream_t st) {
   TcGemmP p = p_in;
   const size_t smem = (size_t)WS_STAGES * (TC_A_BYTES + (size_t)p.BN * TC_BK * 2) + 1024;
-  static SmemOptIn opt, opt_gelu;
+  static SmemOptIn opt, opt_gelu, opt_gate;
   {
-    cudaError_t e = opt.ensure(tc_igemm_ws_kernel<NCOLS, false>, smem, true);
-    if (e == cudaSuccess) e = opt_gelu.ensure(tc_igemm_ws_kernel<NCOLS, true>, smem, true);
+    cudaError_t e = opt.ensure(tc_igemm_ws_kernel<NCOLS, false, false>, smem, true);
+    if (e == cudaSuccess) e = opt_gelu.ensure(tc_igemm_ws_kernel<NCOLS, true, false>, smem, true);
+    if (e == cudaSuccess) e = opt_gate.ensure(tc_igemm_ws_kernel<NCOLS, false, true>, smem, true);
     if (e != cudaSuccess) return (int)e;
   }
   const int tiles = ((p.M + TC_BM - 1) / TC_BM) * ((p.N + p.BN - 1) / p.BN);
@@ -672,6 +718,7 @@
   const int grid = tiles < num_sms * per_sm ? tiles : num_sms * per_sm;
   CUtensorMap tmA, tmW;
   int rc;
+  if (p.gate && (p.conv || p.K % 8 || p.rows_per_img <= 0 || p.act == ACT_GELU)) return (int)cudaErrorInvalidValue;
   p.im2col = 0;
   if (p.conv && p.Wpad && p.Cin <= TC_BK && p.M % (p.OH * p.OW) == 0 && make_tmap_im2col(&tmA, p) == 0) {
     p.im2col = 1;
@@ -686,8 +733,9 @@
   if (getenv("FRX_DEBUG"))
     fprintf(stderr, "[frx] tc gemm M=%d N=%d K=%d BN=%d conv=%d Cin=%d stride=%d -> %s, grid %d\n", p.M, p.N, p.K, p.BN, p.conv,
             p.Cin, p.stride, p.im2col ? "TMA im2col" : (p.conv ? "cp.async gather" : "TMA dense"), grid);
-  if (p.act == ACT_GELU) tc_igemm_ws_kernel<NCOLS, true><<<grid, WS_THREADS, smem, st>>>(p, tmA, tmW);
-  else tc_igemm_ws_kernel<NCOLS, false><<<grid, WS_THREADS, smem, st>>>(p, tmA, tmW);
+  if (p.gate) tc_igemm_ws_kernel<NCOLS, false, true><<<grid, WS_THREADS, smem, st>>>(p, tmA, tmW);
+  else if (p.act == ACT_GELU) tc_igemm_ws_kernel<NCOLS, true, false><<<grid, WS_THREADS, smem, st>>>(p, tmA, tmW);
+  else tc_igemm_ws_kernel<NCOLS, false, false><<<grid, WS_THREADS, smem, st>>>(p, tmA, tmW);
   return 0;
 }
 
@@ -704,6 +752,7 @@
 }
 
 int launch_tc_igemm(TcGemmP p, cudaStream_t st) {
+  if (p.gate) return (int)cudaErrorInvalidValue;
   if (p.act == ACT_GELU) {
     int dev = 0, sms = 148;
     cudaGetDevice(&dev);
diff --git a/p4-fr-sorry-math-but-love-you_b200/csrc/runtime.cu b/p4-fr-sorry-math-but-love-you_b200/csrc/runtime.cu
--- a/p4-fr-sorry-math-but-love-you_b200/csrc/runtime.cu
+++ b/p4-fr-sorry-math-but-love-you_b200/csrc/runtime.cu
@@ -237,6 +237,7 @@
   else if (k == "conv24") h->opt_conv24 = value != 0;
   else if (k == "enc_fp32") h->opt_enc_fp32 = value != 0;
   else if (k == "tc_ws") h->opt_tc_ws = value != 0;
+  else if (k == "se_fused") h->opt_se_fused = value != 0;
   else if (k == "train_splitk") h->opt_train_splitk = value != 0;
   else if (k == "tc_im2col") h->opt_tc_im2col = value != 0;
   else if (k == "prof") {
@@ -821,6 +822,9 @@
       for (int i = 0; i < 2; ++i) { if (dev_alloc(h, &p, B * mid_max * 4)) return 1; h->mid[i] = (float*)p; }
       if (dev_alloc(h, &p, B * 2048 * 4 * 2)) return 1;
       h->gate = (float*)p;
+      if (dev_alloc(h, &p, B * sizeof(int))) return 1;
+      CK(cudaMemset(p, 0, B * sizeof(int)));
+      h->se_arrivals = (int*)p;
     }
     const size_t D = c.dec_hidden, F = c.dec_filter, L = c.dec_layers, T = c.max_steps, V = c.num_classes;
     if (want_dec) {
@@ -1074,12 +1078,15 @@
       int pt, pl;
       same_pad(H, b.k, b.stride, &OH, &pt);
       same_pad(W, b.k, b.stride, &OW, &pl);
-      launch_mbconv_dw_se_bf16(m0, A + b.w_dw, A + b.sc_dw, A + b.sh_dw, m1, h->gate, h->gate + (size_t)B * 2048,
-                               A + b.se_w1, A + b.se_b1, A + b.se_w2t, A + b.se_b2, B, H, W, b.mid, OH, OW, b.stride, pt, pl,
-                               b.se_r, st);
-      CKL(); h->launches += 2;
+      float* gate = h->gate + (size_t)B * 2048;
+      const int nl = launch_mbconv_dw_se_bf16(m0, A + b.w_dw, A + b.sc_dw, A + b.sh_dw, m1, h->gate, gate, A + b.se_w1,
+                                              A + b.se_b1, A + b.se_w2t, A + b.se_b2, B, H, W, b.mid, OH, OW, b.stride, pt,
+                                              pl, b.se_r, h->opt_se_fused && h->opt_tc_ws ? h->se_arrivals : nullptr, st);
+      CKL(); h->launches += nl - 1;
+      if (tap(h, b.name + ".se_gate", gate, B, 1, 1, b.mid, st)) return 1;
       TcGemmP g2 = tc_dense(m1, B * OH * OW, b.mid, A, b.wb_b, b.cout, y, 0);
       g2.scale = A + b.sc_b; g2.shift = A + b.sh_b;
+      if (nl == 1) { g2.gate = gate; g2.rows_per_img = OH * OW; }
       if (b.residual) { g2.res = x; g2.ldr = b.cout; }
       TCL(g2);
     }
diff --git a/p4-fr-sorry-math-but-love-you_b200/csrc/runtime.h b/p4-fr-sorry-math-but-love-you_b200/csrc/runtime.h
--- a/p4-fr-sorry-math-but-love-you_b200/csrc/runtime.h
+++ b/p4-fr-sorry-math-but-love-you_b200/csrc/runtime.h
@@ -79,6 +79,7 @@
   int opt_dec_hpc = 0;
   bool opt_conv24 = true;
   bool opt_enc_fp32 = false;
+  bool opt_se_fused = true;
   long long* prof = nullptr;
   int opt_parts = 3;
   int feat_h = 0, feat_w = 0;
@@ -107,6 +108,7 @@
   size_t dpack2_first = 0;
 
   float *act[2] = {nullptr, nullptr}, *mid[2] = {nullptr, nullptr}, *gate = nullptr;
+  int* se_arrivals = nullptr;
   float *kself = nullptr, *vself = nullptr, *cross = nullptr;
   float *dx = nullptr, *dqkv = nullptr, *datt = nullptr, *dpre1 = nullptr, *dpre2 = nullptr, *du = nullptr,
         *dw = nullptr, *dq2 = nullptr, *dff = nullptr;
```

New measurement: 12470, median of 6. -4.4%, worse.
